# roysubhankar/dwt-domain-adaptation

Measured on NVIDIA H100. Metric: ResNet-50-DWT images/sec fwd+bwd, higher is better.
Workload: dtype f32

## Files before the change

### dwt-domain-adaptation_b200/dwt_b200/_native.py

```python
from __future__ import annotations

import ctypes
import os
import threading

import torch

_HERE = os.path.dirname(os.path.abspath(__file__))
LIB_PATH = os.environ.get("DWT_B200_LIB") or os.path.join(_HERE, "lib", "libdwt_b200.so")

ABI_VERSION = 6
MAX_DOMAINS = 4
MAX_GROUP_SIZE = 64
MODE_TRAIN, MODE_EVAL = 0, 1
EPI_NONE, EPI_AFFINE, EPI_RELU, EPI_RESIDUAL = 0, 1, 2, 4
LAYOUT_NHWC = 0x100
STATUS_NOT_PD, STATUS_BAD_LABEL = 1, 2
KIND_WHITEN, KIND_BN = 0, 1

_c_float_p = ctypes.c_void_p
_PtrArray = ctypes.c_void_p * MAX_DOMAINS


class TailSite(ctypes.Structure):
    _fields_ = [("x", ctypes.c_void_p), ("eps", ctypes.c_float), ("momentum", ctypes.c_float),
                ("update_running", ctypes.c_int), ("running_mean", ctypes.POINTER(ctypes.c_void_p)),
                ("running_cov", ctypes.POINTER(ctypes.c_void_p)), ("gamma", ctypes.c_void_p), ("beta", ctypes.c_void_p),
                ("save_mean", ctypes.c_void_p), ("save_w", ctypes.c_void_p), ("dx", ctypes.c_void_p),
                ("dgamma", ctypes.c_void_p), ("dbeta", ctypes.c_void_p)]

_SIGNATURES = {
    "dwt_abi_version": (ctypes.c_int, []),
    "dwt_last_error": (ctypes.c_char_p, []),
    "dwt_workspace_bytes": (ctypes.c_size_t, [ctypes.c_int64, ctypes.c_int64, ctypes.c_int64, ctypes.c_int, ctypes.c_int]),
    "dwt_whiten_fwd": (ctypes.c_int, [_c_float_p, _c_float_p, ctypes.c_int64, ctypes.c_int64, ctypes.c_int64,
                                      ctypes.c_int, ctypes.c_int, ctypes.c_int, ctypes.c_float, ctypes.c_float,
                                      ctypes.c_int, ctypes.POINTER(ctypes.c_void_p), ctypes.POINTER(ctypes.c_void_p),
                                      _c_float_p, _c_float_p, _c_float_p, ctypes.c_void_p, ctypes.c_int, _c_float_p,
                                      _c_float_p, ctypes.c_void_p, ctypes.c_size_t, ctypes.c_void_p]),
    "dwt_whiten_bwd": (ctypes.c_int, [_c_float_p, _c_float_p, _c_float_p, _c_float_p, ctypes.c_int64, ctypes.c_int64,
                                      ctypes.c_int64, ctypes.c_int, ctypes.c_int, ctypes.c_int, ctypes.c_float,
                                      _c_float_p, _c_float_p, _c_float_p, _c_float_p, ctypes.c_void_p, _c_float_p,
                                      ctypes.c_int, _c_float_p, _c_float_p, ctypes.c_void_p, ctypes.c_size_t,
                                      ctypes.c_void_p]),
    "dwt_bn_fwd": (ctypes.c_int, [_c_float_p, _c_float_p, ctypes.c_int64, ctypes.c_int64, ctypes.c_int64,
                                  ctypes.c_int, ctypes.c_int, ctypes.c_float, ctypes.c_float, ctypes.c_int,
                                  ctypes.POINTER(ctypes.c_void_p), ctypes.POINTER(ctypes.c_void_p), _c_float_p,
                                  _c_float_p, _c_float_p, ctypes.c_void_p, ctypes.c_int, _c_float_p, _c_float_p,
                                  ctypes.c_void_p, ctypes.c_size_t, ctypes.c_void_p]),
    "dwt_bn_bwd": (ctypes.c_int, [_c_float_p, _c_float_p, _c_float_p, _c_float_p, ctypes.c_int64, ctypes.c_int64, ctypes.c_int64,
                                  ctypes.c_int, ctypes.c_int, _c_float_p, _c_float_p, _c_float_p, _c_float_p,
                                  ctypes.c_void_p, _c_float_p, ctypes.c_int, _c_float_p, _c_float_p, ctypes.c_void_p,
                                  ctypes.c_size_t, ctypes.c_void_p]),
    "dwt_tail2_fwd": (ctypes.c_int, [ctypes.c_int, ctypes.POINTER(TailSite), _c_float_p, ctypes.c_void_p, ctypes.c_int64,
                                     ctypes.c_int64, ctypes.c_int64, ctypes.c_int, ctypes.c_int, ctypes.c_void_p,
                                     ctypes.c_size_t, ctypes.c_void_p]),
    "dwt_tail2_bwd": (ctypes.c_int, [ctypes.c_int, ctypes.POINTER(TailSite), _c_float_p, _c_float_p, ctypes.c_void_p,
                                     _c_float_p, ctypes.c_int64, ctypes.c_int64, ctypes.c_int64, ctypes.c_int, ctypes.c_int,
                                     ctypes.c_void_p, ctypes.c_size_t, ctypes.c_void_p]),
    "dwt_mec_fwd_bwd": (ctypes.c_int, [_c_float_p, _c_float_p, ctypes.c_int64, ctypes.c_int64, _c_float_p,
                                       _c_float_p, _c_float_p, ctypes.c_void_p]),
    "dwt_head_loss_fwd_bwd": (ctypes.c_int, [_c_float_p, ctypes.c_void_p, ctypes.c_int64, ctypes.c_int64, ctypes.c_float,
                                             _c_float_p, _c_float_p, ctypes.c_void_p, ctypes.c_void_p]),
    "dwt_augment_pair": (ctypes.c_int, [ctypes.c_void_p, ctypes.c_int64, ctypes.c_int, ctypes.c_int, ctypes.c_int,
                                        ctypes.c_void_p, ctypes.c_void_p, ctypes.c_void_p, _c_float_p,
                                        ctypes.POINTER(ctypes.c_float), ctypes.POINTER(ctypes.c_float), _c_float_p,
                                        _c_float_p, ctypes.c_int, ctypes.c_void_p]),
    "dwt_maxpool_fwd": (ctypes.c_int, [_c_float_p, _c_float_p, ctypes.c_void_p, ctypes.c_int64, ctypes.c_int64, ctypes.c_int64,
                                       ctypes.c_int64, ctypes.c_int, ctypes.c_int, ctypes.c_int, ctypes.c_void_p]),
    "dwt_maxpool_bwd": (ctypes.c_int, [_c_float_p, ctypes.c_void_p, _c_float_p, ctypes.c_int64, ctypes.c_int64, ctypes.c_int64,
                                       ctypes.c_int64, ctypes.c_int, ctypes.c_int, ctypes.c_int, ctypes.c_void_p]),
    "dwt_launch_count": (ctypes.c_int64, []),
    "dwt_profile_begin": (None, []),
    "dwt_profile_end": (ctypes.c_int, [ctypes.c_void_p, ctypes.c_int]),
}


class ProfileEntry(ctypes.Structure):
    _fields_ = [("name", ctypes.c_char * 48), ("launches", ctypes.c_int64), ("ms", ctypes.c_double),
                ("bytes", ctypes.c_double)]


def profile_begin():
    lib().dwt_profile_begin()


def profile_end():
    cap = 1024
    buf = (ProfileEntry * cap)()
    k = lib().dwt_profile_end(ctypes.cast(buf, ctypes.c_void_p), cap)
    return {buf[i].name.decode(): dict(launches=buf[i].launches, ms=buf[i].ms, bytes=buf[i].bytes) for i in range(k)}


def by_family(prof):
    out = {}
    for name, v in prof.items():
        f = out.setdefault(name.split("|")[0], dict(launches=0, ms=0.0, bytes=0.0))
        for k in f:
            f[k] += v[k]
    return out


def launch_count() -> int:
    return int(lib().dwt_launch_count())
EXPORTS = tuple(_SIGNATURES)

_lib = None
_lock = threading.Lock()


class NativeError(RuntimeError):
    pass


def lib() -> ctypes.CDLL:
    global _lib
    if _lib is None:
        with _lock:
            if _lib is None:
                if not os.path.exists(LIB_PATH):
                    raise NativeError(
                        f"{LIB_PATH} is missing: build it with `python {os.path.join(_HERE, 'build.py')}` "
                        "(dwt_b200 has no CPU or PyTorch fallback)")
                handle = ctypes.CDLL(LIB_PATH)
                for name, (res, args) in _SIGNATURES.items():
                    fn = getattr(handle, name)
                    fn.restype, fn.argtypes = res, args
                if handle.dwt_abi_version() != ABI_VERSION:
                    raise NativeError("libdwt_b200.so ABI version mismatch; rebuild it")
                _lib = handle
    return _lib


def channels_last_supported(channels: int, group_size: int) -> bool:
    if group_size not in (1, 2, 4) or channels % 4:
        return False
    c4 = channels // 4
    return c4 & (c4 - 1) == 0


def check(rc: int) -> None:
    if rc != 0:
        raise NativeError(f"libdwt_b200 error {rc}: {lib().dwt_last_error().decode()}")


def ptr(t):
    return None if t is None else ctypes.c_void_p(t.data_ptr())


def ptr_array(tensors):
    arr = _PtrArray()
    for i, t in enumerate(tensors):
        arr[i] = None if t is None else t.data_ptr()
    return ctypes.cast(arr, ctypes.POINTER(ctypes.c_void_p))


def require_cuda(*tensors, any_dtype=False) -> torch.device:
    dev = None
    for t in tensors:
        if t is None:
            continue
        if not t.is_cuda:
            raise NativeError("dwt_b200 runs on CUDA tensors only (no CPU fallback); got a tensor on " + str(t.device))
        if t.dtype != torch.float32 and not any_dtype:
            raise NativeError("dwt_b200 computes in float32; got " + str(t.dtype))
        if dev is None:
            dev = t.device
        elif t.device != dev:
            raise NativeError(f"tensors on different devices: {dev} vs {t.device}")
    return dev


def stream_ptr(device) -> ctypes.c_void_p:
    return ctypes.c_void_p(torch.cuda.current_stream(device).cuda_stream)


_workspaces: dict = {}


def workspace(device, n, c, hw, gs, nd):
    need = lib().dwt_workspace_bytes(n, c, hw, gs, nd)
    if need == 0:
        raise NativeError(f"invalid geometry for workspace: C={c} group_size={gs} domains={nd}")
    key = (device.index, torch.cuda.current_stream(device).cuda_stream)
    buf = _workspaces.get(key)
    if buf is None or buf.numel() < need:
        buf = torch.zeros(max(need, 8 << 20), dtype=torch.uint8, device=device)
        _workspaces[key] = buf
    return buf


def status(device=None) -> int:
    device = torch.device("cuda", torch.cuda.current_device()) if device is None else device
    buf = _workspaces.get((device.index, torch.cuda.current_stream(device).cuda_stream))
    return 0 if buf is None else int(buf[:4].view(torch.int32).item())


def status_all(device=None) -> int:
    device = torch.device("cuda", torch.cuda.current_device()) if device is None else device
    torch.cuda.synchronize(device)
    st = 0
    for (idx, _), buf in _workspaces.items():
        if idx == device.index:
            st |= int(buf[:4].view(torch.int32).item())
    return st


def status_ptr(device):
    return ctypes.c_void_p(workspace(device, 1, 4, 1, 1, 1).data_ptr())


def clear_status(device=None) -> None:
    device = torch.device("cuda", torch.cuda.current_device()) if device is None else device
    buf = _workspaces.get((device.index, torch.cuda.current_stream(device).cuda_stream))
    if buf is not None:
        buf[:4].zero_()


class NotPositiveDefiniteError(torch.linalg.LinAlgError):
    """What the reference's torch.cholesky raises at utils/whitening.py:53, raised late: the kernels never sync the
    host, so the failure is seen at the next poll (raise_on_status) or explicit check_status() call."""


_poll = {"every": 0, "count": 0}


def raise_on_status(every: int = 1) -> None:
    _poll["every"], _poll["count"] = max(0, int(every)), 0


def check_status(device=None) -> None:
    st = status(device)
    if st == 0:
        return
    clear_status(device)
    if st & STATUS_NOT_PD:
        raise NotPositiveDefiniteError(
            "cholesky: a whitening covariance was not positive definite (status word bit 0; the reference raises "
            "from torch.cholesky, utils/whitening.py:53); the affected group's output is NaN and its running-"
            "statistics update was skipped")
    if st & STATUS_BAD_LABEL:
        raise IndexError("head loss: a label was outside [0, num_classes) and is not ignore_index=-100 "
                         "(F.nll_loss asserts here); the row was dropped")
    raise NativeError(f"unknown status bits {st:#x}")


def poll_status(device) -> None:
    if _poll["every"]:
        _poll["count"] += 1
        if _poll["count"] >= _poll["every"]:
            _poll["count"] = 0
            check_status(device)
```

### dwt-domain-adaptation_b200/dwt_b200/csrc/api.cu

```cuda
#include <stdarg.h>
#include <stdio.h>
#include <stdlib.h>

#include <atomic>
#include <mutex>
#include <string>
#include <vector>
#include <string.h>

#include "norm_launch.h"

namespace {

thread_local char g_err[512] = "";

int fail(int code, const char* fmt, ...) {
  va_list ap;
  va_start(ap, fmt);
  vsnprintf(g_err, sizeof(g_err), fmt, ap);
  va_end(ap);
  return code;
}

int check_launch(const char* what) {
  cudaError_t e = cudaPeekAtLastError();
  if (e != cudaSuccess) {
    cudaGetLastError();
    return fail(DWT_E_LAUNCH, "%s: %s", what, cudaGetErrorString(e));
  }
  return DWT_OK;
}

int sm_count() {
  static int n = 0;
  if (n == 0) {
    int dev = 0;
    if (cudaGetDevice(&dev) != cudaSuccess ||
        cudaDeviceGetAttribute(&n, cudaDevAttrMultiProcessorCount, dev) != cudaSuccess || n <= 0)
      n = 132;
  }
  return n;
}

std::atomic<int64_t> g_launches{0};
std::mutex g_prof_mu;
bool g_prof_on = false;
struct ProfRec { char name[48]; cudaEvent_t a, b; double bytes; };
std::vector<ProfRec> g_prof;
std::vector<cudaEvent_t> g_event_pool;

cudaEvent_t take_event() {
  if (!g_event_pool.empty()) { cudaEvent_t e = g_event_pool.back(); g_event_pool.pop_back(); return e; }
  cudaEvent_t e = nullptr;
  cudaEventCreate(&e);
  return e;
}

struct Launch {
  cudaStream_t st; ProfRec rec; bool on;
  Launch(const char* family, const dwt::Geom* gm, double bytes, cudaStream_t s) : st(s), on(false) {
    rec.a = rec.b = nullptr; rec.bytes = bytes;
    if (gm) snprintf(rec.name, sizeof(rec.name), "%s|%d|%d|%d|%d|%d", family, gm->C, gm->HW, gm->GS, gm->D, gm->N);
    else snprintf(rec.name, sizeof(rec.name), "%s", family);
    g_launches.fetch_add(1, std::memory_order_relaxed);
    std::lock_guard<std::mutex> lk(g_prof_mu);
    if (g_prof_on && g_prof.size() < (1u << 18)) {
      on = true; rec.a = take_event(); rec.b = take_event();
      cudaEventRecord(rec.a, st);
    }
  }
  ~Launch() {
    if (!on) return;
    cudaEventRecord(rec.b, st);
    std::lock_guard<std::mutex> lk(g_prof_mu);
    g_prof.push_back(rec);
  }
};

std::once_flag g_tiled_once;
int g_tiled_rc = 0;
int ensure_tiled() {
  std::call_once(g_tiled_once, [] { g_tiled_rc = dwt::tiled_init(); });
  return g_tiled_rc;
}

std::once_flag g_tc_once;
int g_tc_rc = 0;
int ensure_tc() {
  std::call_once(g_tc_once, [] { g_tc_rc = dwt::tc_init(); });
  return g_tc_rc;
}

int tc_chunks(const dwt::Geom& g) {
  const int problems = dwt::tc_superblocks(g) * g.D;
  int n = 2 * sm_count() / problems;
  const int64_t tiles = (int64_t)g.N * ((g.HW + 31) / 32);
  if (n > tiles) n = (int)tiles;
  return n < 1 ? 1 : n;
}

int tc_apply_ctas(const dwt::Geom& g, int per_sm, int tile_px) {
  const int problems = dwt::tc_superblocks(g) * g.D;
  int n = per_sm * sm_count() / problems;
  const int64_t tiles = (int64_t)g.N * ((g.HW + tile_px - 1) / tile_px);
  if (n > tiles) n = (int)tiles;
  return n < 1 ? 1 : n;
}

int env_int(const char* name, int dflt) {
  const char* v = getenv(name);
  return (v && *v) ? atoi(v) : dflt;
}

struct ClPlan { int nred, new_, S, gridy, gz_red, gz_ew; };
ClPlan cl_plan(const dwt::Geom& g, int slots_red, int slots_ew, int unroll_red, int unroll_ew) {
  static const int seq_mb = env_int("DWT_CL_SEQ_MB", 1 << 30);
  const int C4 = g.C / 4, CW = C4 < 256 ? C4 : 256, rpi = 256 / CW, gridy = C4 / CW;
  const long long rows = (long long)g.N * g.HW;
  const double mbytes = 4.0 * (double)g.D * (double)rows * (double)g.C / 1048576.0;
  const bool seq = g.D > 1 && mbytes >= (double)seq_mb;
  ClPlan p;
  p.gridy = gridy;
  p.gz_red = p.gz_ew = seq ? 1 : g.D;
  auto shape = [&](int slots, int unroll, int gz) {
    long long by_work = rows / ((long long)rpi * unroll * 2);
    if (by_work < 1) by_work = 1;
    int cap = slots * sm_count() / (gridy * gz);
    if (cap < 1) cap = 1;
    return (int)(by_work < cap ? by_work : cap);
  };
  p.nred = shape(slots_red, unroll_red, p.gz_red);
  p.new_ = shape(slots_ew, unroll_ew, p.gz_ew);
  p.S = p.nred < 8 ? p.nred : 8;
  return p;
}

inline size_t align_up(size_t v, size_t a) { return (v + a - 1) / a * a; }

enum KernelKind { K_STATS, K_APPLY, K_BWD_REDUCE, K_BWD_APPLY };

int slots_per_sm(KernelKind k, int GS) {
  if (GS > 4) return 2;
  return ((k == K_STATS || k == K_APPLY) && GS < 4) ? 4 : 3;
}

int chunk_cap(int GS, int G, int D) {
  (void)GS;
  const int target = 16 * sm_count();
  int cap = (target + G * D - 1) / (G * D);
  return cap < 1 ? 1 : cap;
}

struct Workspace {
  int* status;
  int* counters;
  int* dom_counter;
  int* dom_counter2;
  float* partial;
  float* save_cov;
  float* coef;
  float* dgb_part;
  float* gram;
  float* shift;
  float* red;
  int* bad;
  size_t bytes;
};

constexpr size_t kMaxGroups = 65536;
constexpr size_t kOffCounters = 256;
constexpr size_t kOffDom1 = kOffCounters + sizeof(int) * DWT_MAX_DOMAINS * kMaxGroups;
constexpr size_t kOffDom2 = kOffDom1 + sizeof(int) * kMaxGroups;
constexpr size_t kOffScratch = kOffDom2 + sizeof(int) * kMaxGroups;

Workspace carve(void* base, int64_t C, int GS, int D, size_t start = kOffScratch) {
  const int G = (int)(C / GS);
  const int cap = chunk_cap(GS, G, D);
  size_t off = start;
  auto take = [&](size_t nbytes) { size_t o = off; off = align_up(off + nbytes, 256); return o; };
  char* b = static_cast<char*>(base);
  Workspace w;
  w.status = reinterpret_cast<int*>(b);
  w.counters = reinterpret_cast<int*>(b + kOffCounters);
  w.dom_counter = reinterpret_cast<int*>(b + kOffDom1);
  w.dom_counter2 = reinterpret_cast<int*>(b + kOffDom2);
  size_t partial_floats = (size_t)D * G * cap * (GS * GS + GS);
  if (GS >= 8 && 64 % GS == 0) {
    const size_t tc = ((size_t)2 * sm_count() + (size_t)((C + 63) / 64) * D) * (64 * 64 + 64);
    if (tc > partial_floats) partial_floats = tc;
  }
  size_t red_floats = 1;
  if (dwt::cl_supports((int)C, GS)) {
    const size_t W = (size_t)dwt::cl_bwd_width((int)C, GS);
    const int C4 = (int)C / 4, gridy = C4 <= 256 ? 1 : C4 / 256;
    const size_t cl = (size_t)D * (3 * sm_count() / gridy + 1) * W;
    if (cl > partial_floats) partial_floats = cl;
    red_floats = (size_t)D * 8 * W;
  }
  w.partial = reinterpret_cast<float*>(b + take(sizeof(float) * partial_floats));
  w.red = reinterpret_cast<float*>(b + take(sizeof(float) * red_floats));
  w.save_cov = reinterpret_cast<float*>(b + take(sizeof(float) * (size_t)D * G * GS * GS));
  w.coef = reinterpret_cast<float*>(b + take(sizeof(float) * (size_t)D * G * dwt::coef_stride(GS)));
  w.dgb_part = reinterpret_cast<float*>(b + take(sizeof(float) * (size_t)D * 2 * C));
  const size_t SBn = (size_t)((C + 63) / 64);
  w.gram = reinterpret_cast<float*>(b + take(sizeof(float) * (size_t)D * SBn * (64 * 64 + 64)));
  w.shift = reinterpret_cast<float*>(b + take(sizeof(float) * (size_t)D * SBn * 64));
  w.bad = reinterpret_cast<int*>(b + take(sizeof(int) * (size_t)D * G));
  w.bytes = off;
  return w;
}

struct Plan {
  dwt::Geom gm;
  dwt::Geom gm_ew;
  int vec;
  int chunks_ew;
  bool small;
};

void shape(dwt::Geom& g, int64_t work_units, KernelKind kind, bool small, int* chunks) {
  const bool reduce = (kind == K_STATS || kind == K_BWD_REDUCE);
  const int slots = slots_per_sm(kind, g.GS) * sm_count();
  const int target = reduce ? slots : 4 * slots;
  g.ppc = 1;
  if (small) {
    while (g.ppc < 8 && (int64_t)((g.G + g.ppc - 1) / g.ppc) * g.D > target) g.ppc <<= 1;
  }
  int n = 1;
  if (g.ppc == 1) {
    n = target / (g.G * g.D);
    const int cap = chunk_cap(g.GS, g.G, g.D);
    if (n > cap) n = cap;
    if (n > work_units) n = (int)work_units;
    if (n < 1) n = 1;
  }
  *chunks = n;
}

int make_plan(Plan& p, KernelKind reduce_kind, KernelKind ew_kind, const void* a0, const void* a1, const void* a2,
              int64_t N, int64_t C, int64_t HW, int GS, int D) {
  if (N <= 0 || C <= 0 || HW <= 0) return fail(DWT_E_INVALID, "empty tensor (N=%lld C=%lld HW=%lld)", (long long)N,
                                               (long long)C, (long long)HW);
  if (GS < 1 || GS > DWT_MAX_GROUP_SIZE) return fail(DWT_E_UNSUPPORTED, "group_size %d outside [1,%d]", GS,
                                                     DWT_MAX_GROUP_SIZE);
  if (C % GS != 0) return fail(DWT_E_INVALID, "channels %lld not divisible by group_size %d", (long long)C, GS);
  if (D < 1 || D > DWT_MAX_DOMAINS) return fail(DWT_E_INVALID, "n_domains %d outside [1,%d]", D, DWT_MAX_DOMAINS);
  if (N * C * HW >= (int64_t)1 << 31 || C / GS > 65535)
    return fail(DWT_E_UNSUPPORTED, "shape too large for 32-bit item indexing");
  dwt::Geom& g = p.gm;
  g.N = (int)N; g.C = (int)C; g.HW = (int)HW; g.GS = GS; g.G = (int)(C / GS); g.D = D;
  g.M = (float)((double)N * (double)HW);
  const uintptr_t bits = (uintptr_t)a0 | (uintptr_t)a1 | (uintptr_t)a2;
  p.vec = (HW % 4 == 0 && bits % 16 == 0) ? 4 : 1;
  p.small = dwt::small_supports(GS);
  int64_t work_units;
  if (p.small) work_units = (N * (HW / p.vec) + dwt::kThreads * 2 - 1) / (dwt::kThreads * 2);
  else work_units = (N * HW + 127) / 128;
  if (work_units < 1) work_units = 1;
  shape(g, work_units, reduce_kind, p.small, &g.nchunks);
  p.gm_ew = g;
  shape(p.gm_ew, work_units, ew_kind, p.small, &p.chunks_ew);
  p.gm_ew.nchunks = g.nchunks;
  return DWT_OK;
}

int check_running(bool need_running, float* const* rmean, float* const* rcov, int D) {
  if (!need_running) return DWT_OK;
  if (!rmean || !rcov) return fail(DWT_E_INVALID, "running buffers required");
  for (int d = 0; d < D; ++d)
    if (!rmean[d] || !rcov[d]) return fail(DWT_E_INVALID, "running buffer of domain %d is null", d);
  return DWT_OK;
}

dwt::FwdFin make_fwd_fin(float a, float b, float momentum, float unbias, int update_running, bool need_running,
                         float* const* rmean, float* const* rcov, float* save_mean, float* save_w, const Workspace& w, int D) {
  dwt::FwdFin fin{};
  fin.a = a; fin.b = b; fin.momentum = momentum; fin.unbias = unbias;
  fin.update_running = update_running;
  fin.save_mean = save_mean; fin.save_w = save_w; fin.save_cov = w.save_cov;
  for (int d = 0; d < D; ++d) { fin.rmean[d] = need_running ? rmean[d] : nullptr; fin.rcov[d] = need_running ? rcov[d] : nullptr; }
  fin.dom_counter = w.dom_counter; fin.status = w.status; fin.bad = w.bad;
  if (need_running && D > 1) {
    bool all_same = true, all_distinct = true;
    for (int d = 1; d < D; ++d) {
      if (rmean[d] != rmean[0] || rcov[d] != rcov[0]) all_same = false;
      for (int e = 0; e < d; ++e)
        if (rmean[d] == rmean[e] || rcov[d] == rcov[e]) all_distinct = false;
    }
    fin.aliased = all_same ? 1 : (all_distinct ? 0 : -1);
  }
  return fin;
}

dwt::BwdFin make_bwd_fin(float a, int mode, int epi, const float* save_mean, const float* save_w, const float* gamma,
                         float* dgamma, float* dbeta, const Workspace& w) {
  dwt::BwdFin fin{};
  fin.a = a; fin.mode = mode; fin.epi = epi;
  fin.save_mean = save_mean; fin.save_w = save_w; fin.gamma = gamma;
  fin.coef = w.coef; fin.dgb_part = w.dgb_part;
  fin.dgamma = (epi & DWT_EPI_AFFINE) ? dgamma : nullptr;
  fin.dbeta = (epi & DWT_EPI_AFFINE) ? dbeta : nullptr;
  fin.dom_counter = w.dom_counter2;
  return fin;
}

int whiten_like_fwd(const float* x, float* y, int64_t N, int64_t C, int64_t HW, int GS, int D, int mode, float a,
                    float b, float momentum, float unbias, int update_running, float* const* rmean,
                    float* const* rcov, const float* gamma, const float* beta, const float* residual,
                    uint8_t* relu_mask, int epi, float* save_mean, float* save_w, void* ws, size_t ws_bytes,
                    cudaStream_t st) {
  const bool nhwc = (mode & DWT_LAYOUT_NHWC) != 0;
  mode &= 0xFF;
  Plan p;
  if (int rc = make_plan(p, K_STATS, K_APPLY, x, y, nullptr, N, C, HW, GS, D)) return rc;
  if (!x || !y || !save_mean || !save_w || !ws) return fail(DWT_E_INVALID, "null pointer argument");
  if (nhwc && !dwt::cl_supports((int)C, GS))
    return fail(DWT_E_UNSUPPORTED, "channels-last layout is built for group_size 1, 2, 4 with C/4 a power of two (C=%lld gs=%d)", (long long)C, GS);
  if (nhwc && (((uintptr_t)x | (uintptr_t)y) % 16 != 0)) return fail(DWT_E_INVALID, "channels-last tensors must be 16-byte aligned");
  if (mode != DWT_MODE_TRAIN && mode != DWT_MODE_EVAL) return fail(DWT_E_INVALID, "bad mode %d", mode);
  if ((epi & DWT_EPI_RELU) && !(epi & DWT_EPI_AFFINE)) return fail(DWT_E_INVALID, "RELU epilogue needs AFFINE");
  if ((epi & DWT_EPI_AFFINE) && (!gamma || !beta)) return fail(DWT_E_INVALID, "AFFINE epilogue needs gamma and beta");
  if ((epi & DWT_EPI_RESIDUAL) && ((epi & 3) != 3 || !residual)) return fail(DWT_E_INVALID, "RESIDUAL epilogue needs AFFINE|RELU and a residual tensor");
  if ((epi & DWT_EPI_RESIDUAL) && (uintptr_t)residual % 16 != 0) return fail(DWT_E_INVALID, "residual must be 16-byte aligned");
  if (relu_mask && !((epi & DWT_EPI_RESIDUAL) && nhwc))
    return fail(DWT_E_UNSUPPORTED, "the ReLU byte map is written by the channels-last RESIDUAL epilogue only");
  if (epi != 0 && !p.small)
    return fail(DWT_E_UNSUPPORTED, "fused gamma/beta/ReLU epilogue is built for group_size 1, 2, 4 (got %d)", GS);
  const bool need_running = (mode == DWT_MODE_EVAL) || update_running;
  if (int rc = check_running(need_running, rmean, rcov, D)) return rc;
  Workspace w = carve(ws, C, GS, D);
  if (w.bytes > ws_bytes) return fail(DWT_E_WORKSPACE, "workspace too small: need %zu bytes, got %zu", w.bytes, ws_bytes);
  if ((uintptr_t)ws % 256 != 0) return fail(DWT_E_WORKSPACE, "workspace must be 256-byte aligned");
  if (!p.small && ensure_tiled() != 0) return fail(DWT_E_LAUNCH, "cudaFuncSetAttribute failed (%d)", g_tiled_rc);

  const dwt::FwdFin fin = make_fwd_fin(a, b, momentum, unbias, mode == DWT_MODE_TRAIN ? update_running : 0, need_running,
                                       rmean, rcov, save_mean, save_w, w, D);

  const double E = 4.0 * (double)D * (double)N * (double)C * (double)HW;
  if (nhwc) {
    const ClPlan cp = cl_plan(p.gm, 3, 3, 8, (epi & DWT_EPI_RESIDUAL) ? 4 : 8);
    if (mode == DWT_MODE_TRAIN) {
      {
        Launch l("cl_stats", &p.gm, E, st);
        dwt::cl_stats(x, p.gm, cp.nred, cp.gz_red, w.partial, w.shift, st);
      }
      if (int rc = check_launch("channels-last statistics kernel")) return rc;
      Launch l("cl_fwd_finalize", &p.gm, 0.0, st);
      dwt::cl_fwd_finalize(w.partial, cp.nred, w.shift, p.gm, fin, st);
    } else {
      Launch l("eval_prep", &p.gm, 0.0, st);
      dwt::small_eval_prep(p.gm, fin, st);
    }
    if (int rc = check_launch("channels-last finalize kernel")) return rc;
    {
      Launch l("cl_apply", &p.gm, ((epi & DWT_EPI_RESIDUAL) ? (relu_mask ? 3.0625 : 3.0) : 2.0) * E, st);
      dwt::cl_apply(x, y, p.gm, cp.new_, cp.gz_ew, epi, save_mean, save_w, gamma, beta, residual, relu_mask, st);
    }
    return check_launch("channels-last apply kernel");
  }
  const bool tc = !p.small && dwt::tc_supports(p.gm, p.vec) && ensure_tc() == 0;
  if (mode == DWT_MODE_TRAIN) {
    Launch l(p.small ? "small_stats" : (tc ? "tc_stats" : "tiled_stats"), &p.gm, E, st);
    if (p.small) dwt::small_stats(x, p.gm, p.vec, fin, w.partial, w.counters, st);
    else if (tc) {
      if (int cr = dwt::tc_stats(x, p.gm, tc_chunks(p.gm), w.shift, w.partial, st))
        return fail(DWT_E_LAUNCH, "cuTensorMapEncodeTiled failed (CUresult %d) x=%p N=%d C=%d HW=%d D=%d", cr, (const void*)x, p.gm.N, p.gm.C, p.gm.HW, p.gm.D);
    } else dwt::tiled_stats(x, p.gm, p.vec, fin, w.partial, w.counters, st);
  } else {
    Launch l("eval_prep", &p.gm, 0.0, st);
    if (p.small) dwt::small_eval_prep(p.gm, fin, st);
    else if (tc) dwt::dense_fwd_factor(nullptr, nullptr, p.gm, fin, st);
    else dwt::tiled_eval_prep(p.gm, fin, st);
  }
  if (tc && mode == DWT_MODE_TRAIN) {
    if (int rc = check_launch("tensor-core statistics kernel")) return rc;
    Launch l("dense_fwd_finalize", &p.gm, 0.0, st);
    dwt::dense_partial_reduce(w.partial, tc_chunks(p.gm), dwt::tc_superblocks(p.gm) * D, w.gram, st);
    dwt::dense_fwd_factor(w.gram, w.shift, p.gm, fin, st);
  }
  if (int rc = check_launch("whitening statistics kernel")) return rc;
  {
    Launch l(p.small ? "small_apply" : (tc ? "tc_apply" : "tiled_apply"), &p.gm, ((epi & DWT_EPI_RESIDUAL) ? 3 : 2) * E, st);
    if (p.small) dwt::small_apply(x, y, p.gm_ew, p.vec, p.chunks_ew, epi, save_mean, save_w, gamma, beta, residual, st);
    else if (tc) {
      if (int cr = dwt::tc_apply(x, y, p.gm, tc_apply_ctas(p.gm, 1, 64), save_mean, save_w, st))
        return fail(DWT_E_LAUNCH, "cuTensorMapEncodeTiled failed (CUresult %d)", cr);
    } else dwt::tiled_apply(x, y, p.gm_ew, p.vec, p.chunks_ew, save_mean, save_w, st);
  }
  return check_launch("whitening apply kernel");
}

int whiten_like_bwd(const float* x, const float* dout, const float* dout2, float* dx, int64_t N, int64_t C, int64_t HW, int GS, int D,
                    int mode, float a, const float* save_mean, const float* save_w, const float* gamma,
                    const float* beta, const uint8_t* relu_mask, float* dresidual, int epi, float* dgamma,
                    float* dbeta, void* ws, size_t ws_bytes, cudaStream_t st) {
  const bool nhwc = (mode & DWT_LAYOUT_NHWC) != 0;
  mode &= 0xFF;
  Plan p;
  if (int rc = make_plan(p, K_BWD_REDUCE, K_BWD_APPLY, x, dout, dx, N, C, HW, GS, D)) return rc;
  if (!x || !dout || !dx || !save_mean || !save_w || !ws) return fail(DWT_E_INVALID, "null pointer argument");
  if (dout2 && (!nhwc || (uintptr_t)dout2 % 16 != 0))
    return fail(nhwc ? DWT_E_INVALID : DWT_E_UNSUPPORTED, "a second gradient addend (dout2) is built for the channels-last "
                "kernels (16-byte aligned tensor); add it to dout otherwise");
  if (nhwc && !dwt::cl_supports((int)C, GS))
    return fail(DWT_E_UNSUPPORTED, "channels-last layout is built for group_size 1, 2, 4 with C/4 a power of two (C=%lld gs=%d)", (long long)C, GS);
  if (nhwc && (((uintptr_t)x | (uintptr_t)dout | (uintptr_t)dx) % 16 != 0)) return fail(DWT_E_INVALID, "channels-last tensors must be 16-byte aligned");
  if (mode != DWT_MODE_TRAIN && mode != DWT_MODE_EVAL) return fail(DWT_E_INVALID, "bad mode %d", mode);
  if ((epi & DWT_EPI_RELU) && !(epi & DWT_EPI_AFFINE)) return fail(DWT_E_INVALID, "RELU epilogue needs AFFINE");
  if ((epi & DWT_EPI_AFFINE) && (!gamma || !beta)) return fail(DWT_E_INVALID, "AFFINE epilogue needs gamma and beta");
  if (epi & DWT_EPI_RESIDUAL) {
    if (!nhwc || !relu_mask || (epi & 3) != 3 || !dresidual)
      return fail(DWT_E_INVALID, "backward of a RESIDUAL forward needs the channels-last layout, AFFINE|RELU, the forward's "
                                 "ReLU byte map and dresidual (or pass dout already masked by (out > 0) with epilogue AFFINE)");
    if ((uintptr_t)dresidual % 16 != 0) return fail(DWT_E_INVALID, "dresidual must be 16-byte aligned");
  } else if (relu_mask || dresidual) {
    return fail(DWT_E_INVALID, "relu_mask / dresidual belong to the RESIDUAL epilogue");
  }
  if ((dgamma == nullptr) != (dbeta == nullptr)) return fail(DWT_E_INVALID, "dgamma and dbeta go together");
  if (epi != 0 && !p.small)
    return fail(DWT_E_UNSUPPORTED, "fused gamma/beta/ReLU epilogue is built for group_size 1, 2, 4 (got %d)", GS);
  Workspace w = carve(ws, C, GS, D);
  if (w.bytes > ws_bytes) return fail(DWT_E_WORKSPACE, "workspace too small: need %zu bytes, got %zu", w.bytes, ws_bytes);
  if ((uintptr_t)ws % 256 != 0) return fail(DWT_E_WORKSPACE, "workspace must be 256-byte aligned");
  if (!p.small && ensure_tiled() != 0) return fail(DWT_E_LAUNCH, "cudaFuncSetAttribute failed (%d)", g_tiled_rc);

  const dwt::BwdFin fin = make_bwd_fin(a, mode, epi, save_mean, save_w, gamma, dgamma, dbeta, w);
  const bool masked = nhwc && (epi & DWT_EPI_RESIDUAL) != 0;

  const bool need_reduce = (mode == DWT_MODE_TRAIN) || (fin.dgamma != nullptr) || masked;
  const double E = 4.0 * (double)D * (double)N * (double)C * (double)HW;
  if (nhwc) {
    const ClPlan cp = cl_plan(p.gm, 2, 2, 4, 4);
    if (need_reduce) {
      {
        Launch l("cl_bwd_reduce", &p.gm, ((masked ? 3.0625 : 2.0) + (dout2 ? 1.0 : 0.0)) * E, st);
        dwt::cl_bwd_reduce(x, dout, dout2, p.gm, cp.nred, cp.gz_red, epi, save_mean, save_w, gamma, beta, relu_mask, dresidual, w.partial, st);
      }
      if (int rc = check_launch("channels-last backward reduction kernel")) return rc;
      Launch l("cl_bwd_finalize", &p.gm, 0.0, st);
      dwt::cl_bwd_finalize(w.partial, cp.nred, p.gm, fin, st);
    } else {
      Launch l("bwd_prep", &p.gm, 0.0, st);
      dwt::small_bwd_prep(p.gm, fin, st);
    }
    if (int rc = check_launch("channels-last backward finalize kernel")) return rc;
    {
      Launch l("cl_bwd_apply", &p.gm, (3.0 + (dout2 && !masked ? 1.0 : 0.0)) * E, st);
      if (masked) dwt::cl_bwd_apply(x, dresidual, nullptr, dx, p.gm, cp.new_, cp.gz_ew, DWT_EPI_AFFINE, w.coef, save_mean, save_w, gamma, beta, st);
      else dwt::cl_bwd_apply(x, dout, dout2, dx, p.gm, cp.new_, cp.gz_ew, epi, w.coef, save_mean, save_w, gamma, beta, st);
    }
    return check_launch("channels-last backward apply kernel");
  }
  const bool tc = !p.small && dwt::tc_supports(p.gm, p.vec) && ensure_tc() == 0;
  if (need_reduce) {
    Launch l(p.small ? "small_bwd_reduce" : (tc ? "tc_bwd_reduce" : "tiled_bwd_reduce"), &p.gm, 2 * E, st);
    if (p.small) dwt::small_bwd_reduce(x, dout, p.gm, p.vec, fin, beta, w.partial, w.counters, st);
    else if (tc) {
      if (int cr = dwt::tc_bwd_reduce(x, dout, p.gm, tc_chunks(p.gm), save_mean, w.partial, st))
        return fail(DWT_E_LAUNCH, "cuTensorMapEncodeTiled failed (CUresult %d) x=%p dout=%p N=%d C=%d HW=%d D=%d", cr, (const void*)x, (const void*)dout, p.gm.N, p.gm.C, p.gm.HW, p.gm.D);
    } else dwt::tiled_bwd_reduce(x, dout, p.gm, p.vec, fin, w.partial, w.counters, st);
  } else {
    Launch l("bwd_prep", &p.gm, 0.0, st);
    if (p.small) dwt::small_bwd_prep(p.gm, fin, st);
    else if (tc) dwt::dense_bwd_coef(nullptr, p.gm, fin, w.shift, st);
    else dwt::tiled_bwd_prep(p.gm, fin, st);
  }
  if (tc && need_reduce) {
    if (int rc = check_launch("tensor-core backward reduction kernel")) return rc;
    Launch l("dense_bwd_finalize", &p.gm, 0.0, st);
    dwt::dense_partial_reduce(w.partial, tc_chunks(p.gm), dwt::tc_superblocks(p.gm) * D, w.gram, st);
    dwt::dense_bwd_coef(w.gram, p.gm, fin, w.shift, st);
  }
  if (int rc = check_launch("whitening backward reduction kernel")) return rc;
  {
    Launch l(p.small ? "small_bwd_apply" : (tc ? "tc_bwd_apply" : "tiled_bwd_apply"), &p.gm, 3 * E, st);
    if (p.small) dwt::small_bwd_apply(x, dout, dx, p.gm_ew, p.vec, p.chunks_ew, epi, w.coef, save_mean, save_w, gamma, beta, st);
    else if (tc) {
      if (int cr = dwt::tc_bwd_apply(x, dout, dx, p.gm, tc_apply_ctas(p.gm, 1, 64), w.coef, save_mean, w.shift, st))
        return fail(DWT_E_LAUNCH, "cuTensorMapEncodeTiled failed (CUresult %d)", cr);
    } else dwt::tiled_bwd_apply(x, dout, dx, p.gm_ew, p.vec, p.chunks_ew, w.coef, st);
  }
  return check_launch("whitening backward apply kernel");
}

struct SiteConst { float a, b, unbias; };
SiteConst site_const(int kind, float eps, int64_t N, int64_t HW) {
  if (kind == DWT_KIND_BN) {
    const double M = (double)N * (double)HW;
    return {1.f, eps, M > 1.0 ? (float)(M / (M - 1.0)) : 1.f};
  }
  return {1.f - eps, eps, 1.f};
}

int tail2_plan(Plan& p, int kind, const dwt_tail_site* s, const void* out, int64_t N, int64_t C, int64_t HW, int GS, int D) {
  if (kind != DWT_KIND_WHITEN && kind != DWT_KIND_BN) return fail(DWT_E_INVALID, "bad kind %d", kind);
  if (kind == DWT_KIND_BN && GS != 1) return fail(DWT_E_INVALID, "batch norm has group_size 1 (got %d)", GS);
  if (!s) return fail(DWT_E_INVALID, "null pointer argument");
  if (int rc = make_plan(p, K_STATS, K_APPLY, s[0].x, s[1].x, out, N, C, HW, GS, D)) return rc;
  if (!dwt::cl_supports((int)C, GS))
    return fail(DWT_E_UNSUPPORTED, "the two-site tail runs on the channels-last kernels: group_size 1, 2, 4 with C/4 a power of two (C=%lld gs=%d)",
                (long long)C, GS);
  for (int k = 0; k < 2; ++k)
    if (!s[k].x || !s[k].gamma || !s[k].beta || !s[k].save_mean || !s[k].save_w || !out) return fail(DWT_E_INVALID, "null pointer argument");
  if ((((uintptr_t)s[0].x | (uintptr_t)s[1].x | (uintptr_t)out) % 16) != 0) return fail(DWT_E_INVALID, "channels-last tensors must be 16-byte aligned");
  return DWT_OK;
}

int tail2_workspace(Workspace (&w)[2], void* ws, size_t ws_bytes, int64_t C, int GS, int D) {
  if (!ws) return fail(DWT_E_INVALID, "null pointer argument");
  w[0] = carve(ws, C, GS, D);
  w[1] = carve(ws, C, GS, D, w[0].bytes);
  if (w[1].bytes > ws_bytes) return fail(DWT_E_WORKSPACE, "workspace too small: need %zu bytes, got %zu", w[1].bytes, ws_bytes);
  if ((uintptr_t)ws % 256 != 0) return fail(DWT_E_WORKSPACE, "workspace must be 256-byte aligned");
  return DWT_OK;
}

int tail2_fwd(int kind, const dwt_tail_site* s, float* y, uint8_t* relu_mask, int64_t N, int64_t C, int64_t HW, int GS, int D,
              void* ws, size_t ws_bytes, cudaStream_t st) {
  Plan p;
  if (int rc = tail2_plan(p, kind, s, y, N, C, HW, GS, D)) return rc;
  if (!relu_mask) return fail(DWT_E_INVALID, "the two-site tail writes the ReLU byte map its backward reads");
  for (int k = 0; k < 2; ++k)
    if (int rc = check_running(s[k].update_running != 0, s[k].running_mean, s[k].running_cov, D)) return rc;
  Workspace w[2];
  if (int rc = tail2_workspace(w, ws, ws_bytes, C, GS, D)) return rc;
  dwt::FwdFin fin[2];
  for (int k = 0; k < 2; ++k) {
    const SiteConst sc = site_const(kind, s[k].eps, N, HW);
    fin[k] = make_fwd_fin(sc.a, sc.b, s[k].momentum, sc.unbias, s[k].update_running, s[k].update_running != 0, s[k].running_mean,
                          s[k].running_cov, s[k].save_mean, s[k].save_w, w[k], D);
  }
  const double E = 4.0 * (double)D * (double)N * (double)C * (double)HW;
  const ClPlan cp = cl_plan(p.gm, 3, 3, 8, 4);
  for (int k = 0; k < 2; ++k) {
    Launch l("cl_stats", &p.gm, E, st);
    dwt::cl_stats(s[k].x, p.gm, cp.nred, cp.gz_red, w[k].partial, w[k].shift, st);
  }
  if (int rc = check_launch("channels-last statistics kernel")) return rc;
  {
    Launch l("cl_tail2_fwd_finalize", &p.gm, 0.0, st);
    dwt::cl_fwd_finalize(w[0].partial, cp.nred, w[0].shift, p.gm, fin[0], st, &fin[1], (size_t)(w[1].partial - w[0].partial),
                         (size_t)(w[1].shift - w[0].shift));
  }
  if (int rc = check_launch("channels-last finalize kernel")) return rc;
  {
    Launch l("cl_tail2_apply", &p.gm, 3.0625 * E, st);
    dwt::cl_tail2_apply(s[0].x, s[1].x, y, p.gm, cp.new_, cp.gz_ew, s[0].save_mean, s[0].save_w, s[0].gamma, s[0].beta,
                        s[1].save_mean, s[1].save_w, s[1].gamma, s[1].beta, relu_mask, st);
  }
  return check_launch("channels-last two-site apply kernel");
}

int tail2_bwd(int kind, const dwt_tail_site* s, const float* dout, const float* dout2, const uint8_t* relu_mask, float* dz,
              int64_t N, int64_t C, int64_t HW, int GS, int D, void* ws, size_t ws_bytes, cudaStream_t st) {
  Plan p;
  if (int rc = tail2_plan(p, kind, s, dz, N, C, HW, GS, D)) return rc;
  if (!dout || !relu_mask || !s[0].dx || !s[1].dx) return fail(DWT_E_INVALID, "null pointer argument");
  if ((((uintptr_t)dout | (uintptr_t)dout2 | (uintptr_t)s[0].dx | (uintptr_t)s[1].dx) % 16) != 0)
    return fail(DWT_E_INVALID, "channels-last tensors must be 16-byte aligned");
  for (int k = 0; k < 2; ++k)
    if ((s[k].dgamma == nullptr) != (s[k].dbeta == nullptr)) return fail(DWT_E_INVALID, "dgamma and dbeta go together");
  Workspace w[2];
  if (int rc = tail2_workspace(w, ws, ws_bytes, C, GS, D)) return rc;
  dwt::BwdFin fin[2];
  for (int k = 0; k < 2; ++k)
    fin[k] = make_bwd_fin(site_const(kind, s[k].eps, N, HW).a, DWT_MODE_TRAIN, k ? DWT_EPI_AFFINE : (DWT_EPI_AFFINE | DWT_EPI_RELU | DWT_EPI_RESIDUAL),
                          s[k].save_mean, s[k].save_w, s[k].gamma, s[k].dgamma, s[k].dbeta, w[k]);
  const double E = 4.0 * (double)D * (double)N * (double)C * (double)HW;
  const ClPlan cp = cl_plan(p.gm, 2, 2, 4, 4);
  {
    Launch l("cl_tail2_bwd_reduce", &p.gm, (4.0625 + (dout2 ? 1.0 : 0.0)) * E, st);
    dwt::cl_tail2_bwd_reduce(s[0].x, s[1].x, dout, dout2, p.gm, cp.nred, cp.gz_red, s[0].save_mean, s[1].save_mean, relu_mask, dz,
                             w[0].partial, (size_t)(w[1].partial - w[0].partial), st);
  }
  if (int rc = check_launch("channels-last two-site backward reduction kernel")) return rc;
  {
    Launch l("cl_tail2_bwd_finalize", &p.gm, 0.0, st);
    dwt::cl_bwd_finalize(w[0].partial, cp.nred, p.gm, fin[0], st, &fin[1], (size_t)(w[1].partial - w[0].partial));
  }
  if (int rc = check_launch("channels-last backward finalize kernel")) return rc;
  {
    Launch l("cl_tail2_bwd_apply", &p.gm, 5.0 * E, st);
    dwt::cl_tail2_bwd_apply(s[0].x, s[1].x, dz, s[0].dx, s[1].dx, p.gm, cp.new_, cp.gz_ew, w[0].coef, w[1].coef, st);
  }
  return check_launch("channels-last two-site backward apply kernel");
}

}

extern "C" {

int dwt_abi_version(void) { return DWT_B200_ABI_VERSION; }

const char* dwt_last_error(void) { return g_err; }

size_t dwt_workspace_bytes(int64_t N, int64_t C, int64_t HW, int group_size, int n_domains) {
  (void)N; (void)HW;
  if (C <= 0 || group_size < 1 || group_size > DWT_MAX_GROUP_SIZE || C % group_size != 0 || n_domains < 1 ||
      n_domains > DWT_MAX_DOMAINS)
    return 0;
  return carve(nullptr, C, group_size, n_domains, carve(nullptr, C, group_size, n_domains).bytes).bytes;
}

int dwt_whiten_fwd(const float* x, float* y, int64_t N, int64_t C, int64_t HW, int group_size, int n_domains,
                   int mode, float eps, float momentum, int update_running, float* const* running_mean,
                   float* const* running_cov, const float* gamma, const float* beta, const float* residual,
                   uint8_t* relu_mask, int epilogue, float* save_mean, float* save_w, void* workspace,
                   size_t workspace_bytes, dwt_stream_t stream) {
  return whiten_like_fwd(x, y, N, C, HW, group_size, n_domains, mode, 1.f - eps, eps, momentum, 1.f, update_running,
                         running_mean, running_cov, gamma, beta, residual, relu_mask, epilogue, save_mean, save_w,
                         workspace, workspace_bytes, (cudaStream_t)stream);
}

int dwt_whiten_bwd(const float* x, const float* dout, const float* dout2, float* dx, int64_t N, int64_t C, int64_t HW, int group_size,
                   int n_domains, int mode, float eps, const float* save_mean, const float* save_w,
                   const float* gamma, const float* beta, const uint8_t* relu_mask, float* dresidual, int epilogue,
                   float* dgamma, float* dbeta, void* workspace, size_t workspace_bytes, dwt_stream_t stream) {
  return whiten_like_bwd(x, dout, dout2, dx, N, C, HW, group_size, n_domains, mode, 1.f - eps, save_mean, save_w, gamma,
                         beta, relu_mask, dresidual, epilogue, dgamma, dbeta, workspace, workspace_bytes,
                         (cudaStream_t)stream);
}

int dwt_bn_fwd(const float* x, float* y, int64_t N, int64_t C, int64_t HW, int n_domains, int mode, float eps,
               float factor, int update_running, float* const* running_mean, float* const* running_var,
               const float* weight, const float* bias, const float* residual, uint8_t* relu_mask, int epilogue,
               float* save_mean, float* save_invstd, void* workspace, size_t workspace_bytes, dwt_stream_t stream) {
  const double M = (double)N * (double)HW;
  const float unbias = M > 1.0 ? (float)(M / (M - 1.0)) : 1.f;
  return whiten_like_fwd(x, y, N, C, HW, 1, n_domains, mode, 1.f, eps, factor, unbias, update_running, running_mean,
                         running_var, weight, bias, residual, relu_mask, epilogue, save_mean, save_invstd, workspace,
                         workspace_bytes, (cudaStream_t)stream);
}

int dwt_bn_bwd(const float* x, const float* dout, const float* dout2, float* dx, int64_t N, int64_t C, int64_t HW, int n_domains,
               int mode, const float* save_mean, const float* save_invstd, const float* weight, const float* bias,
               const uint8_t* relu_mask, float* dresidual, int epilogue, float* dweight, float* dbias, void* workspace,
               size_t workspace_bytes, dwt_stream_t stream) {
  return whiten_like_bwd(x, dout, dout2, dx, N, C, HW, 1, n_domains, mode, 1.f, save_mean, save_invstd, weight, bias,
                         relu_mask, dresidual, epilogue, dweight, dbias, workspace, workspace_bytes,
                         (cudaStream_t)stream);
}

int dwt_tail2_fwd(int kind, const dwt_tail_site* sites, float* y, uint8_t* relu_mask, int64_t N, int64_t C, int64_t HW,
                  int group_size, int n_domains, void* workspace, size_t workspace_bytes, dwt_stream_t stream) {
  return tail2_fwd(kind, sites, y, relu_mask, N, C, HW, group_size, n_domains, workspace, workspace_bytes, (cudaStream_t)stream);
}

int dwt_tail2_bwd(int kind, const dwt_tail_site* sites, const float* dout, const float* dout2, const uint8_t* relu_mask, float* dz,
                  int64_t N, int64_t C, int64_t HW, int group_size, int n_domains, void* workspace, size_t workspace_bytes,
                  dwt_stream_t stream) {
  return tail2_bwd(kind, sites, dout, dout2, relu_mask, dz, N, C, HW, group_size, n_domains, workspace, workspace_bytes,
                   (cudaStream_t)stream);
}

int dwt_mec_fwd_bwd(const float* x, const float* y, int64_t N, int64_t K, float* loss, float* gx, float* gy,
                    dwt_stream_t stream) {
  if (!x || !y || !loss || !gx || !gy) return fail(DWT_E_INVALID, "null pointer argument");
  if (N <= 0 || K <= 0 || N >= (1 << 24) || K >= (1 << 24)) return fail(DWT_E_INVALID, "bad logits shape [%lld,%lld]", (long long)N, (long long)K);
  {
    Launch l("mec", nullptr, 16.0 * (double)N * (double)K, (cudaStream_t)stream);
    dwt::mec_launch(x, y, (int)N, (int)K, loss, gx, gy, (cudaStream_t)stream);
  }
  return check_launch("MEC kernel");
}

int dwt_head_loss_fwd_bwd(const float* logits, const int64_t* labels, int64_t B, int64_t K, float lambda, float* losses,
                          float* grad, int* status, dwt_stream_t stream) {
  if (!logits || !labels || !losses || !grad) return fail(DWT_E_INVALID, "null pointer argument");
  if (B <= 0 || K <= 0 || B >= (1 << 22) || K >= (1 << 24)) return fail(DWT_E_INVALID, "bad logits shape [3*%lld,%lld]", (long long)B, (long long)K);
  {
    Launch l("head_loss", nullptr, 4.0 * 3 * (double)B * (double)K * 2, (cudaStream_t)stream);
    dwt::head_loss_launch(logits, reinterpret_cast<const long long*>(labels), (int)B, (int)K, lambda, losses, grad, status,
                          (cudaStream_t)stream);
  }
  return check_launch("head loss kernel");
}

int dwt_augment_pair(const uint8_t* images, int64_t B, int src_h, int src_w, int crop, const int32_t* crop_plain,
                     const int32_t* crop_aug, const uint8_t* flip, const float* affine, const float* mean,
                     const float* stdv, float* out_plain, float* out_aug, int layout, dwt_stream_t stream) {
  if (!images || !mean || !stdv) return fail(DWT_E_INVALID, "null pointer argument");
  if (!out_plain && !out_aug) return fail(DWT_E_INVALID, "at least one of out_plain / out_aug is needed");
  if (out_plain && !crop_plain) return fail(DWT_E_INVALID, "out_plain needs crop_plain");
  if (out_aug && (!crop_aug || !flip || !affine)) return fail(DWT_E_INVALID, "out_aug needs crop_aug, flip and affine");
  if (B <= 0 || B > 65535 || src_h <= 0 || src_w <= 0 || src_h > 16384 || src_w > 16384)
    return fail(DWT_E_INVALID, "bad image batch [%lld,%d,%d,3]", (long long)B, src_h, src_w);
  if (crop <= 0 || crop > src_h || crop > src_w) return fail(DWT_E_INVALID, "crop %d does not fit %dx%d", crop, src_h, src_w);
  if (layout != 0 && layout != DWT_LAYOUT_NHWC) return fail(DWT_E_INVALID, "layout must be 0 (NCHW) or DWT_LAYOUT_NHWC");
  for (int c = 0; c < 3; ++c)
    if (!(stdv[c] != 0.f)) return fail(DWT_E_INVALID, "std[%d] must be non-zero", c);
  {
    const double px = (double)B * crop * crop;
    Launch l("augment_pair", nullptr, px * 3 * ((out_plain ? 5.0 : 0.0) + (out_aug ? 5.0 : 0.0)), (cudaStream_t)stream);
    dwt::augment_pair_launch(images, (int)B, src_h, src_w, crop, crop_plain, crop_aug, flip, affine, mean, stdv, out_plain,
                             out_aug, layout != 0, (cudaStream_t)stream);
  }
  return check_launch("augmentation kernel");
}

namespace {
int pool_check(int64_t N, int64_t H, int64_t W, int64_t C, int k, int s, int p, int* OH, int* OW) {
  if (N <= 0 || H <= 0 || W <= 0 || C <= 0 || C % 4 != 0) return fail(DWT_E_INVALID, "bad pooling input [%lld,%lld,%lld,%lld] (C must be a multiple of 4)", (long long)N, (long long)H, (long long)W, (long long)C);
  if (k < 1 || k > 15 || s < 1 || p < 0 || 2 * p > k) return fail(DWT_E_INVALID, "bad pooling window k=%d s=%d p=%d (k <= 15, pad <= k/2)", k, s, p);
  if (H + 2 * p < k || W + 2 * p < k) return fail(DWT_E_INVALID, "pooling window larger than the padded image");
  *OH = (int)((H + 2 * p - k) / s + 1);
  *OW = (int)((W + 2 * p - k) / s + 1);
  if (N * H * W * C >= ((int64_t)1 << 40)) return fail(DWT_E_UNSUPPORTED, "tensor too large");
  return DWT_OK;
}
}

int dwt_maxpool_fwd(const float* x, float* y, uint8_t* argmax, int64_t N, int64_t H, int64_t W, int64_t C, int kernel,
                    int stride, int padding, dwt_stream_t stream) {
  int OH = 0, OW = 0;
  if (int rc = pool_check(N, H, W, C, kernel, stride, padding, &OH, &OW)) return rc;
  if (!x || !y || !argmax) return fail(DWT_E_INVALID, "null pointer argument");
  if ((((uintptr_t)x | (uintptr_t)y) % 16) != 0 || (uintptr_t)argmax % 4 != 0) return fail(DWT_E_INVALID, "pooling tensors must be 16-byte aligned");
  {
    const double in = (double)N * H * W * C, out = (double)N * OH * OW * C;
    Launch l("maxpool_fwd", nullptr, 4.0 * (in + out) + out, (cudaStream_t)stream);
    dwt::maxpool_fwd_launch(x, y, argmax, (int)N, (int)H, (int)W, (int)C, OH, OW, kernel, stride, padding, (cudaStream_t)stream);
  }
  return check_launch("max-pool forward kernel");
}

int dwt_maxpool_bwd(const float* dy, const uint8_t* argmax, float* dx, int64_t N, int64_t H, int64_t W, int64_t C, int kernel,
                    int stride, int padding, dwt_stream_t stream) {
  int OH = 0, OW = 0;
  if (int rc = pool_check(N, H, W, C, kernel, stride, padding, &OH, &OW)) return rc;
  if (!dy || !dx || !argmax) return fail(DWT_E_INVALID, "null pointer argument");
  if ((((uintptr_t)dy | (uintptr_t)dx) % 16) != 0 || (uintptr_t)argmax % 4 != 0) return fail(DWT_E_INVALID, "pooling tensors must be 16-byte aligned");
  {
    const double in = (double)N * H * W * C, out = (double)N * OH * OW * C;
    Launch l("maxpool_bwd", nullptr, 4.0 * (in + out) + out, (cudaStream_t)stream);
    dwt::maxpool_bwd_launch(dy, argmax, dx, (int)N, (int)H, (int)W, (int)C, OH, OW, kernel, stride, padding, (cudaStream_t)stream);
  }
  return check_launch("max-pool backward kernel");
}

int64_t dwt_launch_count(void) { return g_launches.load(); }

void dwt_profile_begin(void) {
  std::lock_guard<std::mutex> lk(g_prof_mu);
  for (auto& r : g_prof) { g_event_pool.push_back(r.a); g_event_pool.push_back(r.b); }
  g_prof.clear();
  g_prof_on = true;
}

int dwt_profile_end(dwt_profile_entry* out, int max_entries) {
  std::vector<ProfRec> recs;
  {
    std::lock_guard<std::mutex> lk(g_prof_mu);
    g_prof_on = false;
    recs.swap(g_prof);
  }
  int n = 0;
  for (auto& r : recs) {
    float ms = 0.f;
    if (cudaEventSynchronize(r.b) == cudaSuccess && cudaEventElapsedTime(&ms, r.a, r.b) == cudaSuccess) {
      int k = 0;
      for (; k < n; ++k)
        if (strcmp(out[k].name, r.name) == 0) break;
      if (k == n && n < max_entries) {
        memset(&out[n], 0, sizeof(out[n]));
        strncpy(out[n].name, r.name, sizeof(out[n].name) - 1);
        ++n;
      }
      if (k < n) { out[k].launches += 1; out[k].ms += ms; out[k].bytes += r.bytes; }
    }
    std::lock_guard<std::mutex> lk(g_prof_mu);
    g_event_pool.push_back(r.a); g_event_pool.push_back(r.b);
  }
  return n;
}

}
```

### dwt-domain-adaptation_b200/dwt_b200/csrc/norm_cl.cu

```cuda
#include <stdlib.h>

#include "dwt_common.cuh"
#include "norm_launch.h"
#include "small_algebra.cuh"

namespace dwt {
namespace {

constexpr int kT = 256;

__device__ __forceinline__ void pdl_wait() { asm volatile("griddepcontrol.wait;" ::: "memory"); }
__device__ __forceinline__ void pdl_launch_dependents() { asm volatile("griddepcontrol.launch_dependents;" ::: "memory"); }

template <int GS> struct ClShape {
  static constexpr int NSUB = 4 / GS;
  static constexpr int NM = GS * (GS + 1) / 2;
  static constexpr int FWD1 = GS + NM;
  static constexpr int BWD1 = GS * GS + GS;
  static constexpr int FWD = NSUB * FWD1;
  static constexpr int BWD = NSUB * BWD1;
};

struct ClThread {
  int C4, CW, rpi, col, rsub, q;
  __device__ __forceinline__ ClThread(const Geom& gm) {
    C4 = gm.C >> 2;
    CW = C4 < kT ? C4 : kT;
    rpi = kT / CW;
    col = threadIdx.x % CW;
    rsub = threadIdx.x / CW;
    q = blockIdx.y * CW + col;
  }
};

template <int UNROLL, bool DESC, class F>
__device__ __forceinline__ void sweep_rows(const ClThread& t, unsigned rows, F&& body) {
  const unsigned krows = (unsigned)t.rpi * UNROLL, nch = (rows + krows - 1) / krows;
  for (unsigned i = blockIdx.x; i < nch; i += gridDim.x) body((DESC ? nch - 1 - i : i) * krows + t.rsub);
}
#define CL_FOR_DOMAINS(d, gm, DESC) \
  for (int di_ = blockIdx.z, d = (DESC) ? (gm).D - 1 - di_ : di_; di_ < (gm).D; di_ += gridDim.z, d = (DESC) ? (gm).D - 1 - di_ : di_)

__device__ __forceinline__ float4 ldg4(const float* p) { return __ldg(reinterpret_cast<const float4*>(p)); }

template <int NACC>
__device__ __forceinline__ void column_reduce(const ClThread& t, float (&acc)[NACC], float* sRed) {
  if (t.rpi == 1) return;
#pragma unroll
  for (int i = 0; i < NACC; ++i) sRed[i * kT + threadIdx.x] = acc[i];
  __syncthreads();
  if (t.rsub == 0) {
#pragma unroll
    for (int i = 0; i < NACC; ++i) {
      float s = acc[i];
      for (int r = 1; r < t.rpi; ++r) s += sRed[i * kT + r * t.CW + t.col];
      acc[i] = s;
    }
  }
}

template <int GS>
__global__ void __launch_bounds__(kT, 3) cl_stats_kernel(const float* __restrict__ x, const Geom gm,
                                                         float* __restrict__ partial, float* __restrict__ shift) {
  using S = ClShape<GS>;
  constexpr int UNROLL = 8;
  __shared__ float sRed[kT * S::FWD];
  const ClThread t(gm);
  const unsigned rows = (unsigned)gm.N * gm.HW;
  pdl_launch_dependents();
  CL_FOR_DOMAINS(d, gm, true) {
    const float* xd = x + (size_t)d * rows * gm.C + 4 * t.q;
    float K[4] = {0.f, 0.f, 0.f, 0.f};
    {
      const unsigned np = rows < 8 ? rows : 8;
      for (unsigned r = 0; r < np; ++r) {
        const float4 v = ldg4(xd + (size_t)r * gm.C);
        K[0] += v.x; K[1] += v.y; K[2] += v.z; K[3] += v.w;
      }
#pragma unroll
      for (int c = 0; c < 4; ++c) K[c] /= (float)np;
      if (blockIdx.x == 0 && t.rsub == 0) *reinterpret_cast<float4*>(shift + (size_t)d * gm.C + 4 * t.q) = make_float4(K[0], K[1], K[2], K[3]);
    }
    float acc[S::FWD];
#pragma unroll
    for (int i = 0; i < S::FWD; ++i) acc[i] = 0.f;
    sweep_rows<UNROLL, true>(t, rows, [&](unsigned r) {
      float4 v[UNROLL];
#pragma unroll
      for (int u = 0; u < UNROLL; ++u) {
        const unsigned rr = r + u * t.rpi;
        v[u] = rr < rows ? ldg4(xd + (size_t)rr * gm.C) : make_float4(K[0], K[1], K[2], K[3]);
      }
#pragma unroll
      for (int u = 0; u < UNROLL; ++u) {
        const float e[4] = {v[u].x - K[0], v[u].y - K[1], v[u].z - K[2], v[u].w - K[3]};
#pragma unroll
        for (int s = 0; s < S::NSUB; ++s) {
#pragma unroll
          for (int c = 0; c < GS; ++c) {
            acc[s * S::FWD1 + c] += e[s * GS + c];
#pragma unroll
            for (int j = 0; j <= c; ++j)
              acc[s * S::FWD1 + GS + c * (c + 1) / 2 + j] = fmaf(e[s * GS + c], e[s * GS + j], acc[s * S::FWD1 + GS + c * (c + 1) / 2 + j]);
          }
        }
      }
    });
    column_reduce<S::FWD>(t, acc, sRed);
    if (t.rsub == 0) {
      float* dst = partial + (((size_t)d * gridDim.x + blockIdx.x) * t.C4 + t.q) * S::FWD;
#pragma unroll
      for (int i = 0; i < S::FWD; ++i) dst[i] = acc[i];
    }
    if (gridDim.z == 1) __syncthreads();
  }
}

template <int GS, int PER>
__device__ __forceinline__ int acc_index(int g, int a) {
  constexpr int NSUB = 4 / GS;
  return (g / NSUB) * (NSUB * PER) + (g % NSUB) * PER + a;
}

constexpr int kFinQ = 2;

template <int NACC>
__device__ __forceinline__ void column_row_sum(const float* __restrict__ col, int nrows, int W, float (&a)[NACC]) {
  static_assert(NACC % 2 == 0, "accumulators are read as float2");
#pragma unroll
  for (int i = 0; i < NACC; ++i) a[i] = 0.f;
#pragma unroll 4
  for (int r = threadIdx.x; r < nrows; r += 32) {
    const float2* p = reinterpret_cast<const float2*>(col + (size_t)r * W);
#pragma unroll
    for (int i = 0; i < NACC / 2; ++i) {
      const float2 v = __ldcg(p + i);
      a[2 * i] += v.x; a[2 * i + 1] += v.y;
    }
  }
#pragma unroll
  for (int o = 1; o < 32; o <<= 1)
#pragma unroll
    for (int i = 0; i < NACC; ++i) a[i] += __shfl_xor_sync(0xffffffffu, a[i], o);
}

template <int NSUB, int PER>
__device__ __forceinline__ void take_group(const float (&a)[NSUB * PER], int s, float (&v)[PER]) {
#pragma unroll
  for (int i = 0; i < PER; ++i) {
    v[i] = a[i];
#pragma unroll
    for (int k = 1; k < NSUB; ++k)
      if (s == k) v[i] = a[k * PER + i];
  }
}

template <int GS>
__device__ __forceinline__ void cl_fwd_finalize_site(const float* __restrict__ partial, int nrows, const float* __restrict__ shift,
                                                     const Geom& gm, const FwdFin& fin) {
  using SH = ClShape<GS>;
  constexpr int NST = GS + GS * GS;
  __shared__ float sStat[DWT_MAX_DOMAINS][kFinQ][SH::NSUB][NST + 1];
  __shared__ unsigned char sBad[DWT_MAX_DOMAINS][kFinQ][SH::NSUB];
  const int s = threadIdx.x, ql = threadIdx.y, d = threadIdx.z, q = blockIdx.x * blockDim.y + ql;
  const int W = (gm.C >> 2) * SH::FWD;
  const float invM = 1.f / gm.M;
  const bool lead = s < SH::NSUB;
  const int g = q * SH::NSUB + (lead ? s : 0);
  const bool direct = gm.D == 1 || fin.aliased == 0;
  const int dbuf = direct ? d : 0;
  const bool upd = fin.update_running && lead && (direct || (fin.aliased == 1 && d == 0));
  float rc_old[GS * GS], rm_old[GS];
  if (upd) {
#pragma unroll
    for (int e = 0; e < GS * GS; ++e) rc_old[e] = fin.rcov[dbuf][(size_t)g * GS * GS + e];
#pragma unroll
    for (int e = 0; e < GS; ++e) rm_old[e] = fin.rmean[dbuf][g * GS + e];
  }
  pdl_launch_dependents();
  pdl_wait();
  float a[SH::FWD];
  column_row_sum<SH::FWD>(partial + (size_t)d * nrows * W + (size_t)q * SH::FWD, nrows, W, a);
  if (lead) {
    float v[SH::FWD1];
    take_group<SH::NSUB, SH::FWD1>(a, s, v);
    float mean[GS], cov[GS][GS];
#pragma unroll
    for (int i = 0; i < GS; ++i) mean[i] = shift[(size_t)d * gm.C + g * GS + i] + v[i] * invM;
#pragma unroll
    for (int i = 0; i < GS; ++i)
#pragma unroll
      for (int j = 0; j <= i; ++j) {
        const float c = v[GS + i * (i + 1) / 2 + j] * invM - (v[i] * invM) * (v[j] * invM);
        cov[i][j] = c; cov[j][i] = c;
      }
    const bool bad = factor_thread<GS>(gm, fin, d, g, mean, cov, false);
    if (fin.update_running) {
      if (direct) {
        if (!bad) {
          const float m = fin.momentum, kk = 1.f - fin.momentum;
#pragma unroll
          for (int i = 0; i < GS; ++i) {
            fin.rmean[d][g * GS + i] = m * mean[i] + kk * rm_old[i];
#pragma unroll
            for (int j = 0; j < GS; ++j)
              fin.rcov[d][(size_t)g * GS * GS + i * GS + j] = m * (cov[i][j] * fin.unbias) + kk * rc_old[i * GS + j];
          }
        }
      } else {
        sBad[d][ql][s] = bad ? 1 : 0;
#pragma unroll
        for (int i = 0; i < GS; ++i) {
          sStat[d][ql][s][i] = mean[i];
#pragma unroll
          for (int j = 0; j < GS; ++j) sStat[d][ql][s][GS + i * GS + j] = cov[i][j];
        }
      }
    }
  }
  if (!fin.update_running || direct) return;
  __syncthreads();
  if (!(lead && d == 0)) return;
  if (fin.aliased == 1) {
    const float m = fin.momentum, kk = 1.f - fin.momentum;
    float* rc = fin.rcov[0] + (size_t)g * GS * GS;
    float* rm = fin.rmean[0] + g * GS;
    for (int dd = 0; dd < gm.D; ++dd) {
      if (sBad[dd][ql][s]) continue;
#pragma unroll
      for (int e = 0; e < GS * GS; ++e) rc_old[e] = m * (sStat[dd][ql][s][GS + e] * fin.unbias) + kk * rc_old[e];
#pragma unroll
      for (int e = 0; e < GS; ++e) rm_old[e] = m * sStat[dd][ql][s][e] + kk * rm_old[e];
    }
#pragma unroll
    for (int e = 0; e < GS * GS; ++e) rc[e] = rc_old[e];
#pragma unroll
    for (int e = 0; e < GS; ++e) rm[e] = rm_old[e];
  } else {
    for (int dd = 0; dd < gm.D; ++dd)
      if (!sBad[dd][ql][s]) ema_direct<GS>(gm, fin, dd, g, &sStat[dd][ql][s][0], &sStat[dd][ql][s][GS]);
  }
}

template <int GS>
__global__ void __launch_bounds__(32 * kFinQ * DWT_MAX_DOMAINS) cl_fwd_finalize_kernel(const float* __restrict__ partial, size_t pstride, int nrows,
                                                                                      const float* __restrict__ shift, size_t sstride, const Geom gm,
                                                                                      const __grid_constant__ FwdFin fin, const __grid_constant__ FwdFin fin2) {
  const bool second = blockIdx.y != 0;
  cl_fwd_finalize_site<GS>(partial + (second ? pstride : 0), nrows, shift + (second ? sstride : 0), gm, second ? fin2 : fin);
}

template <int GS, int EPI, bool DS>
__global__ void __launch_bounds__(kT, 3) cl_apply_kernel(const float* __restrict__ x, float* __restrict__ y, const Geom gm,
                                                         const float* __restrict__ save_mean, const float* __restrict__ save_w,
                                                         const float* __restrict__ gamma, const float* __restrict__ beta,
                                                         const float* __restrict__ res, uint8_t* __restrict__ mask,
                                                         const float* __restrict__ save_mean_d, const float* __restrict__ save_w_d,
                                                         const float* __restrict__ gamma_d, const float* __restrict__ beta_d) {
  using S = ClShape<GS>;
  constexpr bool RES = (EPI & DWT_EPI_RESIDUAL) != 0;
  static_assert(!DS || RES, "the two-site tail is a residual epilogue");
  constexpr int UNROLL = DS ? 2 : (RES ? 4 : 8);
  const ClThread t(gm);
  const unsigned rows = (unsigned)gm.N * gm.HW;
  pdl_wait();
  CL_FOR_DOMAINS(d, gm, false) {
    float Wp[S::NSUB][S::NM], bp[S::NSUB][GS], Wd[DS ? S::NSUB : 1][S::NM], bd[DS ? S::NSUB : 1][GS];
#pragma unroll
    for (int s = 0; s < S::NSUB; ++s) {
      const int g = t.q * S::NSUB + s;
      load_forward_map<GS, EPI>(save_w + ((size_t)d * gm.G + g) * GS * GS, save_mean + (size_t)d * gm.C + g * GS,
                                gamma + g * GS, beta + g * GS, Wp[s], bp[s]);
      if constexpr (DS)
        load_forward_map<GS, DWT_EPI_AFFINE>(save_w_d + ((size_t)d * gm.G + g) * GS * GS, save_mean_d + (size_t)d * gm.C + g * GS,
                                             gamma_d + g * GS, beta_d + g * GS, Wd[s], bd[s]);
    }
    const size_t base = (size_t)d * rows * gm.C + 4 * t.q;
    const float* xd = x + base;
    const float* rd = res + base;
    float* yd = y + base;
    uint8_t* md = mask + (size_t)d * rows * t.C4 + t.q;
    sweep_rows<UNROLL, false>(t, rows, [&](unsigned r) {
      float4 v[UNROLL], rs[UNROLL];
#pragma unroll
      for (int u = 0; u < UNROLL; ++u) {
        const unsigned rr = r + u * t.rpi;
        if (rr < rows) {
          v[u] = ldg4(xd + (size_t)rr * gm.C);
          if constexpr (RES) rs[u] = ldg4(rd + (size_t)rr * gm.C);
        }
      }
#pragma unroll
      for (int u = 0; u < UNROLL; ++u) {
        const unsigned rr = r + u * t.rpi;
        if (rr < rows) {
          const float e[4] = {v[u].x, v[u].y, v[u].z, v[u].w};
          float o[4], ra[4] = {0.f, 0.f, 0.f, 0.f};
          if constexpr (RES) { ra[0] = rs[u].x; ra[1] = rs[u].y; ra[2] = rs[u].z; ra[3] = rs[u].w; }
          unsigned bits = 0;
#pragma unroll
          for (int s = 0; s < S::NSUB; ++s) {
            float xi[GS], oi[GS];
            if constexpr (DS) {
              float xdi[GS], odi[GS];
#pragma unroll
              for (int c = 0; c < GS; ++c) xdi[c] = ra[s * GS + c];
              apply_group<GS>(Wd[s], bd[s], xdi, odi);
#pragma unroll
              for (int c = 0; c < GS; ++c) ra[s * GS + c] = odi[c];
            }
#pragma unroll
            for (int c = 0; c < GS; ++c) xi[c] = e[s * GS + c];
            apply_group<GS>(Wp[s], bp[s], xi, oi);
#pragma unroll
            for (int c = 0; c < GS; ++c) {
              const float z = RES ? oi[c] + ra[s * GS + c] : oi[c];
              if constexpr (RES) bits |= (z > 0.f ? 1u : 0u) << (s * GS + c);
              o[s * GS + c] = (EPI & DWT_EPI_RELU) ? fmaxf(z, 0.f) : z;
            }
          }
          *reinterpret_cast<float4*>(yd + (size_t)rr * gm.C) = make_float4(o[0], o[1], o[2], o[3]);
          if constexpr (RES) { if (mask != nullptr) md[(size_t)rr * t.C4] = (uint8_t)bits; }
        }
      }
    });
  }
}

template <int GS>
__device__ __forceinline__ void bwd_accumulate(float* acc, const float (&dz)[GS], const float (&xi)[GS], const float* mu) {
#pragma unroll
  for (int i = 0; i < GS; ++i) {
    acc[GS * GS + i] += dz[i];
#pragma unroll
    for (int j = 0; j < GS; ++j) acc[i * GS + j] = fmaf(dz[i], xi[j] - mu[j], acc[i * GS + j]);
  }
}

template <int GS, int EPI, bool D2, bool DS>
__global__ void __launch_bounds__(kT, 2) cl_bwd_reduce_kernel(const float* __restrict__ x, const float* __restrict__ dout, const float* __restrict__ dout2,
                                                              const Geom gm, const float* __restrict__ save_mean,
                                                              const float* __restrict__ save_w, const float* __restrict__ gamma,
                                                              const float* __restrict__ beta, const uint8_t* __restrict__ mask,
                                                              float* __restrict__ dzout, float* __restrict__ partial,
                                                              const float* __restrict__ xds, const float* __restrict__ save_mean_d,
                                                              size_t pstride) {
  using S = ClShape<GS>;
  constexpr int UNROLL = 4;
  constexpr bool MASK = (EPI & DWT_EPI_RESIDUAL) != 0;
  constexpr bool RELU = (EPI & DWT_EPI_RELU) != 0 && !MASK;
  static_assert(!DS || MASK, "the two-site tail is a residual epilogue");
  constexpr int NS = DS ? 2 : 1;
  __shared__ float sRed[kT * S::BWD];
  const ClThread t(gm);
  const unsigned rows = (unsigned)gm.N * gm.HW;
  pdl_launch_dependents();
  CL_FOR_DOMAINS(d, gm, true) {
    float Wp[S::NSUB][S::NM], bp[S::NSUB][GS], mu[NS][4];
#pragma unroll
    for (int s = 0; s < S::NSUB; ++s) {
      const int g = t.q * S::NSUB + s;
      if constexpr (RELU)
        load_forward_map<GS, EPI>(save_w + ((size_t)d * gm.G + g) * GS * GS, save_mean + (size_t)d * gm.C + g * GS,
                                  gamma + g * GS, beta + g * GS, Wp[s], bp[s]);
    }
#pragma unroll
    for (int k = 0; k < NS; ++k) {
      const float4 m4 = ldg4((k ? save_mean_d : save_mean) + (size_t)d * gm.C + 4 * t.q);
      mu[k][0] = m4.x; mu[k][1] = m4.y; mu[k][2] = m4.z; mu[k][3] = m4.w;
    }
    float acc[NS][S::BWD];
#pragma unroll
    for (int k = 0; k < NS; ++k)
#pragma unroll
      for (int i = 0; i < S::BWD; ++i) acc[k][i] = 0.f;
    const size_t base = (size_t)d * rows * gm.C + 4 * t.q;
    const float* xp[NS];
    xp[0] = x + base;
    if constexpr (DS) xp[NS - 1] = xds + base;
    const float* gd = dout + base;
    const float* gd2 = D2 ? dout2 + base : nullptr;
    float* zd = MASK ? dzout + base : nullptr;
    const uint8_t* md = mask + (size_t)d * rows * t.C4 + t.q;
    constexpr int H = DS ? UNROLL / 2 : UNROLL;
    sweep_rows<UNROLL, true>(t, rows, [&](unsigned r0) {
#pragma unroll
     for (int h = 0; h < UNROLL; h += H) {
      const unsigned r = r0 + h * t.rpi;
      float4 v[NS][H], q[H], q2[D2 ? H : 1];
      unsigned mb[H];
#pragma unroll
      for (int u = 0; u < H; ++u) {
        const unsigned rr = r + u * t.rpi;
        if (rr < rows) {
#pragma unroll
          for (int k = 0; k < NS; ++k) v[k][u] = ldg4(xp[k] + (size_t)rr * gm.C);
          q[u] = ldg4(gd + (size_t)rr * gm.C);
          if constexpr (MASK) mb[u] = __ldg(md + (size_t)rr * t.C4);
          if constexpr (D2) q2[u] = ldg4(gd2 + (size_t)rr * gm.C);
        } else {
#pragma unroll
          for (int k = 0; k < NS; ++k) v[k][u] = make_float4(mu[k][0], mu[k][1], mu[k][2], mu[k][3]);
          q[u] = make_float4(0.f, 0.f, 0.f, 0.f);
          if constexpr (MASK) mb[u] = 0u;
          if constexpr (D2) q2[u] = make_float4(0.f, 0.f, 0.f, 0.f);
        }
      }
      if constexpr (D2) {
#pragma unroll
        for (int u = 0; u < H; ++u) { q[u].x += q2[u].x; q[u].y += q2[u].y; q[u].z += q2[u].z; q[u].w += q2[u].w; }
      }
#pragma unroll
      for (int u = 0; u < H; ++u) {
        const float ge[4] = {q[u].x, q[u].y, q[u].z, q[u].w};
        const float e[4] = {v[0][u].x, v[0][u].y, v[0][u].z, v[0][u].w};
        const float ed[4] = {v[NS - 1][u].x, v[NS - 1][u].y, v[NS - 1][u].z, v[NS - 1][u].w};
        float zm[4];
#pragma unroll
        for (int s = 0; s < S::NSUB; ++s) {
          float xi[GS], dz[GS];
#pragma unroll
          for (int c = 0; c < GS; ++c) { xi[c] = e[s * GS + c]; dz[c] = ge[s * GS + c]; }
          if constexpr (RELU) {
            float oi[GS];
            apply_group<GS>(Wp[s], bp[s], xi, oi);
#pragma unroll
            for (int c = 0; c < GS; ++c) dz[c] = oi[c] > 0.f ? dz[c] : 0.f;
          }
          if constexpr (MASK) {
#pragma unroll
            for (int c = 0; c < GS; ++c) { dz[c] = ((mb[u] >> (s * GS + c)) & 1u) ? dz[c] : 0.f; zm[s * GS + c] = dz[c]; }
          }
          bwd_accumulate<GS>(acc[0] + s * S::BWD1, dz, xi, &mu[0][s * GS]);
          if constexpr (DS) {
#pragma unroll
            for (int c = 0; c < GS; ++c) xi[c] = ed[s * GS + c];
            bwd_accumulate<GS>(acc[NS - 1] + s * S::BWD1, dz, xi, &mu[NS - 1][s * GS]);
          }
        }
        if constexpr (MASK) {
          const unsigned rr = r + u * t.rpi;
          if (rr < rows) *reinterpret_cast<float4*>(zd + (size_t)rr * gm.C) = make_float4(zm[0], zm[1], zm[2], zm[3]);
        }
      }
     }
    });
#pragma unroll
    for (int k = 0; k < NS; ++k) {
      if (k) __syncthreads();
      column_reduce<S::BWD>(t, acc[k], sRed);
      if (t.rsub == 0) {
        float* dst = partial + k * pstride + (((size_t)d * gridDim.x + blockIdx.x) * t.C4 + t.q) * S::BWD;
#pragma unroll
        for (int i = 0; i < S::BWD; ++i) dst[i] = acc[k][i];
      }
    }
    if (gridDim.z == 1) __syncthreads();
  }
}

template <int GS>
__device__ __forceinline__ void cl_bwd_finalize_site(const float* __restrict__ partial, int nrows, const Geom& gm, const BwdFin& fin) {
  using SH = ClShape<GS>;
  const int s = threadIdx.x, d = threadIdx.z, q = blockIdx.x * blockDim.y + threadIdx.y;
  const int W = (gm.C >> 2) * SH::BWD;
  pdl_launch_dependents();
  pdl_wait();
  float a[SH::BWD];
  column_row_sum<SH::BWD>(partial + (size_t)d * nrows * W + (size_t)q * SH::BWD, nrows, W, a);
  if (s < SH::NSUB) {
    float v[SH::BWD1], R[GS][GS], sdz[GS];
    take_group<SH::NSUB, SH::BWD1>(a, s, v);
#pragma unroll
    for (int i = 0; i < SH::BWD1; ++i) {
      if (i < GS * GS) R[i / GS][i % GS] = v[i]; else sdz[i - GS * GS] = v[i];
    }
    bwd_finalize_thread<GS>(gm, fin, d, q * SH::NSUB + s, R, sdz, false);
  }
  if (!((fin.epi & DWT_EPI_AFFINE) && fin.dgamma != nullptr)) return;
  __syncthreads();
  if (d == 0 && s < 4) {
    const int ch = 4 * q + s;
    float sg = 0.f, sb = 0.f;
    for (int dd = 0; dd < gm.D; ++dd) {
      sg += fin.dgb_part[((size_t)dd * 2 + 0) * gm.C + ch];
      sb += fin.dgb_part[((size_t)dd * 2 + 1) * gm.C + ch];
    }
    fin.dgamma[ch] = sg;
    fin.dbeta[ch] = sb;
  }
}

template <int GS>
__global__ void __launch_bounds__(32 * kFinQ * DWT_MAX_DOMAINS) cl_bwd_finalize_kernel(const float* __restrict__ partial, size_t pstride, int nrows,
                                                                                      const Geom gm, const __grid_constant__ BwdFin fin,
                                                                                      const __grid_constant__ BwdFin fin2) {
  const bool second = blockIdx.y != 0;
  cl_bwd_finalize_site<GS>(partial + (second ? pstride : 0), nrows, gm, second ? fin2 : fin);
}

template <int GS>
struct BwdCoef {
  float A1[GS * (GS + 1) / 2], Bm[GS * (GS + 1) / 2], cv[GS];
  __device__ __forceinline__ void load(const float* cf) {
#pragma unroll
    for (int i = 0; i < GS; ++i) {
      cv[i] = __ldg(cf + 2 * GS * GS + i);
#pragma unroll
      for (int j = 0; j <= i; ++j) {
        A1[i * (i + 1) / 2 + j] = __ldg(cf + j * GS + i);
        Bm[i * (i + 1) / 2 + j] = __ldg(cf + GS * GS + i * GS + j);
      }
    }
  }
  __device__ __forceinline__ void apply(const float (&dz)[GS], const float (&xi)[GS], float* o) const {
#pragma unroll
    for (int i = 0; i < GS; ++i) {
      float a = cv[i];
#pragma unroll
      for (int j = i; j < GS; ++j) a = fmaf(A1[j * (j + 1) / 2 + i], dz[j], a);
#pragma unroll
      for (int j = 0; j < GS; ++j) {
        const int hi = i > j ? i : j, lo = i > j ? j : i;
        a = fmaf(Bm[hi * (hi + 1) / 2 + lo], xi[j], a);
      }
      o[i] = a;
    }
  }
};

template <int GS, int EPI, bool D2, bool DS>
__global__ void __launch_bounds__(kT, 2) cl_bwd_apply_kernel(const float* __restrict__ x, const float* __restrict__ dout, const float* __restrict__ dout2,
                                                             float* __restrict__ dx, const Geom gm, const float* __restrict__ coef,
                                                             const float* __restrict__ save_mean, const float* __restrict__ save_w,
                                                             const float* __restrict__ gamma, const float* __restrict__ beta,
                                                             const float* __restrict__ xds, float* __restrict__ dxds,
                                                             const float* __restrict__ coef_d) {
  using S = ClShape<GS>;
  constexpr int UNROLL = 4;
  constexpr bool RELU = (EPI & DWT_EPI_RELU) != 0;
  static_assert((EPI & DWT_EPI_RESIDUAL) == 0, "the residual tail's apply runs with EPI = AFFINE on dz");
  static_assert(!DS || (!D2 && !RELU), "the two-site tail's apply reads dz");
  constexpr int NS = DS ? 2 : 1;
  const ClThread t(gm);
  const unsigned rows = (unsigned)gm.N * gm.HW;
  pdl_wait();
  CL_FOR_DOMAINS(d, gm, false) {
    float Wp[S::NSUB][S::NM], bp[S::NSUB][GS];
    BwdCoef<GS> cf[NS][S::NSUB];
#pragma unroll
    for (int s = 0; s < S::NSUB; ++s) {
      const int g = t.q * S::NSUB + s;
      if constexpr (RELU)
        load_forward_map<GS, EPI>(save_w + ((size_t)d * gm.G + g) * GS * GS, save_mean + (size_t)d * gm.C + g * GS,
                                  gamma + g * GS, beta + g * GS, Wp[s], bp[s]);
#pragma unroll
      for (int k = 0; k < NS; ++k) cf[k][s].load((k ? coef_d : coef) + ((size_t)d * gm.G + g) * coef_stride(GS));
    }
    const size_t base = (size_t)d * rows * gm.C + 4 * t.q;
    const float* xp[NS];
    float* op[NS];
    xp[0] = x + base; op[0] = dx + base;
    if constexpr (DS) { xp[NS - 1] = xds + base; op[NS - 1] = dxds + base; }
    const float* gd = dout + base;
    const float* gd2 = D2 ? dout2 + base : nullptr;
    sweep_rows<UNROLL, false>(t, rows, [&](unsigned r) {
      float4 v[NS][UNROLL], q[UNROLL], q2[D2 ? UNROLL : 1];
#pragma unroll
      for (int u = 0; u < UNROLL; ++u) {
        const unsigned rr = r + u * t.rpi;
        if (rr < rows) {
#pragma unroll
          for (int k = 0; k < NS; ++k) v[k][u] = ldg4(xp[k] + (size_t)rr * gm.C);
          q[u] = ldg4(gd + (size_t)rr * gm.C);
          if constexpr (D2) q2[u] = ldg4(gd2 + (size_t)rr * gm.C);
        }
      }
      if constexpr (D2) {
#pragma unroll
        for (int u = 0; u < UNROLL; ++u)
          if (r + u * t.rpi < rows) { q[u].x += q2[u].x; q[u].y += q2[u].y; q[u].z += q2[u].z; q[u].w += q2[u].w; }
      }
#pragma unroll
      for (int u = 0; u < UNROLL; ++u) {
        const unsigned rr = r + u * t.rpi;
        if (rr < rows) {
          const float ge[4] = {q[u].x, q[u].y, q[u].z, q[u].w};
#pragma unroll
          for (int k = 0; k < NS; ++k) {
            const float e[4] = {v[k][u].x, v[k][u].y, v[k][u].z, v[k][u].w};
            float o[4];
#pragma unroll
            for (int s = 0; s < S::NSUB; ++s) {
              float xi[GS], dz[GS];
#pragma unroll
              for (int c = 0; c < GS; ++c) { xi[c] = e[s * GS + c]; dz[c] = ge[s * GS + c]; }
              if constexpr (RELU) {
                float oi[GS];
                apply_group<GS>(Wp[s], bp[s], xi, oi);
#pragma unroll
                for (int c = 0; c < GS; ++c) dz[c] = oi[c] > 0.f ? dz[c] : 0.f;
              }
              cf[k][s].apply(dz, xi, o + s * GS);
            }
            *reinterpret_cast<float4*>(op[k] + (size_t)rr * gm.C) = make_float4(o[0], o[1], o[2], o[3]);
          }
        }
      }
    });
  }
}

#define CL_GS(GS_, ...)                                  \
  switch (GS_) {                                         \
    case 1: { constexpr int kGS = 1; __VA_ARGS__; break; } \
    case 2: { constexpr int kGS = 2; __VA_ARGS__; break; } \
    case 4: { constexpr int kGS = 4; __VA_ARGS__; break; } \
    default: break;                                      \
  }
#define CL_EPI(E_, ...)                                                   \
  if ((E_) == 3) { constexpr int kEPI = 3; __VA_ARGS__; }                 \
  else if ((E_) == 1) { constexpr int kEPI = 1; __VA_ARGS__; }            \
  else { constexpr int kEPI = 0; __VA_ARGS__; }
#define CL_EPI_BWD(E_, ...)                                               \
  if ((E_) == 7) { constexpr int kEPI = 7; __VA_ARGS__; }                 \
  else CL_EPI(E_, __VA_ARGS__)
#define CL_D2(P_, ...)                                                    \
  if (P_) { constexpr bool kD2 = true; __VA_ARGS__; }                     \
  else { constexpr bool kD2 = false; __VA_ARGS__; }

inline bool use_pdl() {
  static const bool on = [] { const char* v = getenv("DWT_PDL"); return v != nullptr && v[0] == '1'; }();
  return on;
}

template <class... KArgs, class... Args>
inline void launch_k(void (*kernel)(KArgs...), dim3 grid, dim3 block, cudaStream_t st, bool pdl, Args... args) {
  cudaLaunchConfig_t cfg = {};
  cfg.gridDim = grid; cfg.blockDim = block; cfg.dynamicSmemBytes = 0; cfg.stream = st;
  cudaLaunchAttribute attr[1];
  attr[0].id = cudaLaunchAttributeProgrammaticStreamSerialization;
  attr[0].val.programmaticStreamSerializationAllowed = 1;
  cfg.attrs = attr; cfg.numAttrs = pdl ? 1 : 0;
  cudaLaunchKernelEx(&cfg, kernel, KArgs(args)...);
}

inline dim3 cl_grid(const Geom& gm, int nctas, int gz) {
  const int C4 = gm.C / 4, CW = C4 < kT ? C4 : kT;
  return dim3(nctas, C4 / CW, gz);
}

}

bool cl_supports(int C, int GS) {
  if (!(GS == 1 || GS == 2 || GS == 4) || C % 4 != 0) return false;
  const int c4 = C / 4;
  return (c4 & (c4 - 1)) == 0 && c4 <= 16384;
}
int cl_fwd_width(int C, int GS) { return (C / 4) * (4 / GS) * (GS + GS * (GS + 1) / 2); }
int cl_bwd_width(int C, int GS) { return (C / 4) * (4 / GS) * (GS * GS + GS); }


void cl_stats(const float* x, const Geom& gm, int nctas, int gz, float* partial, float* shift, cudaStream_t st) {
  CL_GS(gm.GS, (cl_stats_kernel<kGS><<<cl_grid(gm, nctas, gz), kT, 0, st>>>(x, gm, partial, shift)));
}
inline dim3 fin_block(const Geom& gm) { const int c4 = gm.C / 4; return dim3(32, c4 < kFinQ ? c4 : kFinQ, gm.D); }
void cl_fwd_finalize(const float* partial, int nrows, const float* shift, const Geom& gm, const FwdFin& fin, cudaStream_t st,
                     const FwdFin* fin2, size_t pstride, size_t sstride) {
  const dim3 b = fin_block(gm), g((gm.C / 4) / b.y, fin2 ? 2 : 1);
  CL_GS(gm.GS, (launch_k(cl_fwd_finalize_kernel<kGS>, g, b, st, use_pdl(), partial, pstride, nrows, shift, sstride, gm, fin, fin2 ? *fin2 : fin)));
}
void cl_apply(const float* x, float* y, const Geom& gm, int nctas, int gz, int epi, const float* mean, const float* w,
              const float* gamma, const float* beta, const float* residual, uint8_t* mask, cudaStream_t st) {
  const float* nul = nullptr;
  if (epi == 7) {
    CL_GS(gm.GS, (launch_k(cl_apply_kernel<kGS, 7, false>, cl_grid(gm, nctas, gz), dim3(kT), st, use_pdl(), x, y, gm, mean, w, gamma, beta, residual, mask,
                           nul, nul, nul, nul)));
    return;
  }
  CL_GS(gm.GS, CL_EPI(epi, (launch_k(cl_apply_kernel<kGS, kEPI, false>, cl_grid(gm, nctas, gz), dim3(kT), st, use_pdl(), x, y, gm, mean, w, gamma, beta,
                                     nul, (uint8_t*)nullptr, nul, nul, nul, nul))));
}
void cl_tail2_apply(const float* x, const float* xd, float* y, const Geom& gm, int nctas, int gz, const float* mean, const float* w,
                    const float* gamma, const float* beta, const float* mean_d, const float* w_d, const float* gamma_d,
                    const float* beta_d, uint8_t* mask, cudaStream_t st) {
  CL_GS(gm.GS, (launch_k(cl_apply_kernel<kGS, 7, true>, cl_grid(gm, nctas, gz), dim3(kT), st, use_pdl(), x, y, gm, mean, w, gamma, beta, xd, mask,
                         mean_d, w_d, gamma_d, beta_d)));
}
void cl_bwd_reduce(const float* x, const float* dout, const float* dout2, const Geom& gm, int nctas, int gz, int epi, const float* mean, const float* w,
                   const float* gamma, const float* beta, const uint8_t* mask, float* dz, float* partial, cudaStream_t st) {
  const float* nul = nullptr;
  CL_GS(gm.GS, CL_D2(dout2, CL_EPI_BWD(epi, (cl_bwd_reduce_kernel<kGS, kEPI, kD2, false><<<cl_grid(gm, nctas, gz), kT, 0, st>>>(
                                                x, dout, dout2, gm, mean, w, gamma, beta, mask, dz, partial, nul, nul, 0)))));
}
void cl_tail2_bwd_reduce(const float* x, const float* xd, const float* dout, const float* dout2, const Geom& gm, int nctas, int gz,
                         const float* mean, const float* mean_d, const uint8_t* mask, float* dz, float* partial, size_t pstride,
                         cudaStream_t st) {
  const float* nul = nullptr;
  CL_GS(gm.GS, CL_D2(dout2, (cl_bwd_reduce_kernel<kGS, 7, kD2, true><<<cl_grid(gm, nctas, gz), kT, 0, st>>>(
                                x, dout, dout2, gm, mean, nul, nul, nul, mask, dz, partial, xd, mean_d, pstride))));
}
void cl_bwd_finalize(const float* partial, int nrows, const Geom& gm, const BwdFin& fin, cudaStream_t st, const BwdFin* fin2, size_t pstride) {
  const dim3 b = fin_block(gm), g((gm.C / 4) / b.y, fin2 ? 2 : 1);
  CL_GS(gm.GS, (launch_k(cl_bwd_finalize_kernel<kGS>, g, b, st, use_pdl(), partial, pstride, nrows, gm, fin, fin2 ? *fin2 : fin)));
}
void cl_bwd_apply(const float* x, const float* dout, const float* dout2, float* dx, const Geom& gm, int nctas, int gz, int epi, const float* coef,
                  const float* mean, const float* w, const float* gamma, const float* beta, cudaStream_t st) {
  const float* nul = nullptr;
  CL_GS(gm.GS, CL_D2(dout2, CL_EPI(epi, (launch_k(cl_bwd_apply_kernel<kGS, kEPI, kD2, false>, cl_grid(gm, nctas, gz), dim3(kT), st, use_pdl(), x, dout,
                                                  dout2, dx, gm, coef, mean, w, gamma, beta, nul, (float*)nullptr, nul)))));
}
void cl_tail2_bwd_apply(const float* x, const float* xd, const float* dz, float* dx, float* dxd, const Geom& gm, int nctas, int gz,
                        const float* coef, const float* coef_d, cudaStream_t st) {
  const float* nul = nullptr;
  CL_GS(gm.GS, (launch_k(cl_bwd_apply_kernel<kGS, 1, false, true>, cl_grid(gm, nctas, gz), dim3(kT), st, use_pdl(), x, dz, nul, dx, gm, coef,
                         nul, nul, nul, nul, xd, dxd, coef_d)));
}

}
```

### dwt-domain-adaptation_b200/dwt_b200/csrc/norm_launch.h

```cpp
#pragma once
#include <stdint.h>

#include "dwt_common.cuh"

namespace dwt {

inline void bind_context() {
  thread_local bool bound = false;
  if (!bound) { cudaFree(nullptr); bound = true; }
}

bool small_supports(int GS);
void small_stats(const float* x, const Geom& gm, int vec, const FwdFin& fin, float* partial, int* counters,
                 cudaStream_t st);
void small_eval_prep(const Geom& gm, const FwdFin& fin, cudaStream_t st);
void small_apply(const float* x, float* y, const Geom& gm, int vec, int chunks, int epi, const float* mean,
                 const float* w, const float* gamma, const float* beta, const float* residual, cudaStream_t st);
void small_bwd_reduce(const float* x, const float* dout, const Geom& gm, int vec, const BwdFin& fin,
                      const float* beta, float* partial, int* counters, cudaStream_t st);
void small_bwd_prep(const Geom& gm, const BwdFin& fin, cudaStream_t st);
void small_bwd_apply(const float* x, const float* dout, float* dx, const Geom& gm, int vec, int chunks, int epi,
                     const float* coef, const float* mean, const float* w, const float* gamma, const float* beta,
                     cudaStream_t st);

int tiled_smem_bytes(int GS);
int tiled_init();
void tiled_stats(const float* x, const Geom& gm, int vec, const FwdFin& fin, float* partial, int* counters,
                 cudaStream_t st);
void tiled_eval_prep(const Geom& gm, const FwdFin& fin, cudaStream_t st);
void tiled_apply(const float* x, float* y, const Geom& gm, int vec, int chunks, const float* mean, const float* w,
                 cudaStream_t st);
void tiled_bwd_reduce(const float* x, const float* dout, const Geom& gm, int vec, const BwdFin& fin, float* partial,
                      int* counters, cudaStream_t st);
void tiled_bwd_prep(const Geom& gm, const BwdFin& fin, cudaStream_t st);
void tiled_bwd_apply(const float* x, const float* dout, float* dx, const Geom& gm, int vec, int chunks,
                     const float* coef, cudaStream_t st);

int tc_init();
bool tc_supports(const Geom& gm, int vec);
int tc_superblocks(const Geom& gm);
int tc_stats(const float* x, const Geom& gm, int nchunks, float* shift, float* partial, cudaStream_t st);
int tc_bwd_reduce(const float* x, const float* dout, const Geom& gm, int nchunks, const float* save_mean,
                  float* partial, cudaStream_t st);

int dense_init();
void dense_partial_reduce(const float* partial, int nchunks, int problems, float* gram, cudaStream_t st);
void dense_fwd_factor(const float* gram, const float* shift, const Geom& gm, const FwdFin& fin, cudaStream_t st);
void dense_bwd_coef(const float* rgram, const Geom& gm, const BwdFin& fin, float* dybar, cudaStream_t st);

int tc_apply_init();
int tc_apply(const float* x, float* y, const Geom& gm, int nctas, const float* save_mean, const float* save_w,
             cudaStream_t st);
int tc_bwd_apply(const float* x, const float* dout, float* dx, const Geom& gm, int nctas, const float* coef,
                 const float* save_mean, const float* dybar, cudaStream_t st);

bool cl_supports(int C, int GS);
int cl_fwd_width(int C, int GS);
int cl_bwd_width(int C, int GS);
void cl_stats(const float* x, const Geom& gm, int nctas, int gz, float* partial, float* shift, cudaStream_t st);
void cl_fwd_finalize(const float* partial, int nrows, const float* shift, const Geom& gm, const FwdFin& fin, cudaStream_t st,
                     const FwdFin* fin2 = nullptr, size_t pstride = 0, size_t sstride = 0);
void cl_apply(const float* x, float* y, const Geom& gm, int nctas, int gz, int epi, const float* mean, const float* w,
              const float* gamma, const float* beta, const float* residual, uint8_t* mask, cudaStream_t st);
void cl_bwd_reduce(const float* x, const float* dout, const float* dout2, const Geom& gm, int nctas, int gz, int epi, const float* mean, const float* w,
                   const float* gamma, const float* beta, const uint8_t* mask, float* dz, float* partial, cudaStream_t st);
void cl_bwd_finalize(const float* partial, int nrows, const Geom& gm, const BwdFin& fin, cudaStream_t st,
                     const BwdFin* fin2 = nullptr, size_t pstride = 0);
void cl_bwd_apply(const float* x, const float* dout, const float* dout2, float* dx, const Geom& gm, int nctas, int gz, int epi, const float* coef,
                  const float* mean, const float* w, const float* gamma, const float* beta, cudaStream_t st);
void cl_tail2_apply(const float* x, const float* xd, float* y, const Geom& gm, int nctas, int gz, const float* mean, const float* w,
                    const float* gamma, const float* beta, const float* mean_d, const float* w_d, const float* gamma_d,
                    const float* beta_d, uint8_t* mask, cudaStream_t st);
void cl_tail2_bwd_reduce(const float* x, const float* xd, const float* dout, const float* dout2, const Geom& gm, int nctas, int gz,
                         const float* mean, const float* mean_d, const uint8_t* mask, float* dz, float* partial, size_t pstride,
                         cudaStream_t st);
void cl_tail2_bwd_apply(const float* x, const float* xd, const float* dz, float* dx, float* dxd, const Geom& gm, int nctas, int gz,
                        const float* coef, const float* coef_d, cudaStream_t st);

void maxpool_fwd_launch(const float* x, float* y, uint8_t* idx, int N, int H, int W, int C, int OH, int OW, int k, int s, int p,
                        cudaStream_t st);
void maxpool_bwd_launch(const float* dy, const uint8_t* idx, float* dx, int N, int H, int W, int C, int OH, int OW, int k, int s,
                        int p, cudaStream_t st);

void augment_pair_launch(const uint8_t* images, int B, int SH, int SW, int CR, const int* crop_plain, const int* crop_aug,
                         const uint8_t* flip, const float* affine, const float* mean, const float* stdv,
                         float* out_plain, float* out_aug, int nhwc, cudaStream_t st);
void head_loss_launch(const float* logits, const long long* labels, int B, int K, float lambda, float* losses,
                      float* grad, int* status, cudaStream_t st);
void mec_launch(const float* x, const float* y, int N, int K, float* loss, float* gx, float* gy, cudaStream_t st);

}
```

### dwt-domain-adaptation_b200/dwt_b200/csrc/pool.cu

```cuda
#include "dwt_common.cuh"
#include "norm_launch.h"

namespace dwt {
namespace {

struct PoolGeom {
  int N, H, W, C4, OH, OW, k, s, p, c4shift;
};

template <int K, int S, int P>
__device__ __forceinline__ PoolGeom fixed(PoolGeom g) {
  if constexpr (K > 0) { g.k = K; g.s = S; g.p = P; }
  return g;
}

__device__ __forceinline__ bool takes(float v, float best) { return (v > best) || (v != v); }

template <int K, int S, int P, bool POW2>
__global__ void __launch_bounds__(256) maxpool_fwd_kernel(const float* __restrict__ x, float* __restrict__ y,
                                                          uint8_t* __restrict__ idx, const PoolGeom g0) {
  const PoolGeom g = fixed<K, S, P>(g0);
  const int n = blockIdx.x / g.OH, oh = blockIdx.x - n * g.OH;
  const int h0 = oh * g.s - g.p;
  const float4* xn = reinterpret_cast<const float4*>(x) + (size_t)n * g.H * g.W * g.C4;
  const size_t obase = ((size_t)n * g.OH + oh) * g.OW * g.C4;
  for (int t = threadIdx.x; t < g.OW * g.C4; t += blockDim.x) {
    const int ow = POW2 ? (t >> g.c4shift) : t / g.C4, c4 = t - ow * g.C4;
    const int w0 = ow * g.s - g.p;
    float best[4] = {-INFINITY, -INFINITY, -INFINITY, -INFINITY};
    unsigned bi[4] = {0u, 0u, 0u, 0u};
#pragma unroll
    for (int kh = 0; kh < g.k; ++kh) {
      const int h = h0 + kh;
      if (h < 0 || h >= g.H) continue;
      const float4* xr = xn + (size_t)h * g.W * g.C4 + c4;
#pragma unroll
      for (int kw = 0; kw < g.k; ++kw) {
        const int w = w0 + kw;
        if (w < 0 || w >= g.W) continue;
        const float4 v = __ldg(xr + (size_t)w * g.C4);
        const float e[4] = {v.x, v.y, v.z, v.w};
        const unsigned code = (unsigned)(kh * g.k + kw);
#pragma unroll
        for (int c = 0; c < 4; ++c)
          if (takes(e[c], best[c])) { best[c] = e[c]; bi[c] = code; }
      }
    }
    reinterpret_cast<float4*>(y)[obase + t] = make_float4(best[0], best[1], best[2], best[3]);
    reinterpret_cast<uint32_t*>(idx)[obase + t] = bi[0] | (bi[1] << 8) | (bi[2] << 16) | (bi[3] << 24);
  }
}

template <int K, int S, int P, bool POW2>
__global__ void __launch_bounds__(256) maxpool_bwd_kernel(const float* __restrict__ dy, const uint8_t* __restrict__ idx,
                                                          float* __restrict__ dx, const PoolGeom g0) {
  const PoolGeom g = fixed<K, S, P>(g0);
  const int n = blockIdx.x / g.H, h = blockIdx.x - n * g.H;
  int oh0 = h + g.p - g.k + 1;
  oh0 = oh0 <= 0 ? 0 : (oh0 + g.s - 1) / g.s;
  int oh1 = (h + g.p) / g.s;
  if (oh1 > g.OH - 1) oh1 = g.OH - 1;
  const float4* dyn = reinterpret_cast<const float4*>(dy) + (size_t)n * g.OH * g.OW * g.C4;
  const uint32_t* ixn = reinterpret_cast<const uint32_t*>(idx) + (size_t)n * g.OH * g.OW * g.C4;
  float4* dxr = reinterpret_cast<float4*>(dx) + ((size_t)n * g.H + h) * g.W * g.C4;
  for (int t = threadIdx.x; t < g.W * g.C4; t += blockDim.x) {
    const int w = POW2 ? (t >> g.c4shift) : t / g.C4, c4 = t - w * g.C4;
    int ow0 = w + g.p - g.k + 1;
    ow0 = ow0 <= 0 ? 0 : (ow0 + g.s - 1) / g.s;
    int ow1 = (w + g.p) / g.s;
    if (ow1 > g.OW - 1) ow1 = g.OW - 1;
    float acc[4] = {0.f, 0.f, 0.f, 0.f};
    for (int oh = oh0; oh <= oh1; ++oh) {
      const unsigned kh = (unsigned)(h - (oh * g.s - g.p));
      for (int ow = ow0; ow <= ow1; ++ow) {
        const unsigned code = kh * g.k + (unsigned)(w - (ow * g.s - g.p));
        const size_t o = ((size_t)oh * g.OW + ow) * g.C4 + c4;
        const uint32_t m = __ldg(ixn + o);
        const bool h0 = (m & 0xFFu) == code, h1 = ((m >> 8) & 0xFFu) == code, h2 = ((m >> 16) & 0xFFu) == code, h3 = (m >> 24) == code;
        if (h0 || h1 || h2 || h3) {
          const float4 gq = __ldg(dyn + o);
          if (h0) acc[0] += gq.x;
          if (h1) acc[1] += gq.y;
          if (h2) acc[2] += gq.z;
          if (h3) acc[3] += gq.w;
        }
      }
    }
    dxr[t] = make_float4(acc[0], acc[1], acc[2], acc[3]);
  }
}

__global__ void __launch_bounds__(256) maxpool_fwd_3s2_kernel(const float* __restrict__ x, float* __restrict__ y,
                                                              uint8_t* __restrict__ idx, const PoolGeom g) {
  const int OH2 = g.OH >> 1, OW2 = g.OW >> 1;
  const int n = blockIdx.y / OH2, a = blockIdx.y - n * OH2;
  const int i = blockIdx.x * blockDim.x + threadIdx.x;
  if (i >= OW2 * g.C4) return;
  const int b = i >> g.c4shift, c4 = i & (g.C4 - 1);
  const float4* xn = reinterpret_cast<const float4*>(x) + (size_t)n * g.H * g.W * g.C4 + c4;
  float best[2][2][4];
  unsigned bi[2][2][4];
#pragma unroll
  for (int oa = 0; oa < 2; ++oa)
#pragma unroll
    for (int ob = 0; ob < 2; ++ob)
#pragma unroll
      for (int c = 0; c < 4; ++c) { best[oa][ob][c] = -INFINITY; bi[oa][ob][c] = 0u; }
  const int h0 = 4 * a - 1, w0 = 4 * b - 1;
#pragma unroll
  for (int r = 0; r < 5; ++r) {
    const int h = h0 + r;
    if (h < 0 || h >= g.H) continue;
    float4 row[5];
    bool in[5];
#pragma unroll
    for (int cc = 0; cc < 5; ++cc) {
      const int w = w0 + cc;
      in[cc] = w >= 0 && w < g.W;
      row[cc] = in[cc] ? __ldg(xn + ((size_t)h * g.W + w) * g.C4) : make_float4(0.f, 0.f, 0.f, 0.f);
    }
#pragma unroll
    for (int oa = 0; oa < 2; ++oa) {
      const int kh = r - 2 * oa;
      if (kh < 0 || kh > 2) continue;
#pragma unroll
      for (int ob = 0; ob < 2; ++ob)
#pragma unroll
        for (int kw = 0; kw < 3; ++kw) {
          const int cc = 2 * ob + kw;
          if (!in[cc]) continue;
          const float e[4] = {row[cc].x, row[cc].y, row[cc].z, row[cc].w};
          const unsigned code = (unsigned)(kh * 3 + kw);
#pragma unroll
          for (int c = 0; c < 4; ++c)
            if (takes(e[c], best[oa][ob][c])) { best[oa][ob][c] = e[c]; bi[oa][ob][c] = code; }
        }
    }
  }
#pragma unroll
  for (int oa = 0; oa < 2; ++oa)
#pragma unroll
    for (int ob = 0; ob < 2; ++ob) {
      const size_t o = (((size_t)n * g.OH + 2 * a + oa) * g.OW + 2 * b + ob) * g.C4 + c4;
      reinterpret_cast<float4*>(y)[o] = make_float4(best[oa][ob][0], best[oa][ob][1], best[oa][ob][2], best[oa][ob][3]);
      reinterpret_cast<uint32_t*>(idx)[o] = bi[oa][ob][0] | (bi[oa][ob][1] << 8) | (bi[oa][ob][2] << 16) | (bi[oa][ob][3] << 24);
    }
}

__device__ __forceinline__ void take(float4& acc, const float4& gq, uint32_t m, unsigned code) {
  if ((m & 0xFFu) == code) acc.x += gq.x;
  if (((m >> 8) & 0xFFu) == code) acc.y += gq.y;
  if (((m >> 16) & 0xFFu) == code) acc.z += gq.z;
  if ((m >> 24) == code) acc.w += gq.w;
}

__global__ void __launch_bounds__(256) maxpool_bwd_3s2_kernel(const float* __restrict__ dy, const uint8_t* __restrict__ idx,
                                                              float* __restrict__ dx, const PoolGeom g) {
  const int H2 = g.H >> 1, W2 = g.W >> 1;
  const int n = blockIdx.y / H2, k = blockIdx.y - n * H2;
  const int i = blockIdx.x * blockDim.x + threadIdx.x;
  if (i >= W2 * g.C4) return;
  const int j = i >> g.c4shift, c4 = i & (g.C4 - 1);
  const float4* dyn = reinterpret_cast<const float4*>(dy) + (size_t)n * g.OH * g.OW * g.C4;
  const uint32_t* ixn = reinterpret_cast<const uint32_t*>(idx) + (size_t)n * g.OH * g.OW * g.C4;
  uint32_t m[2][2];
  float4 gq[2][2];
#pragma unroll
  for (int a = 0; a < 2; ++a)
#pragma unroll
    for (int b = 0; b < 2; ++b) {
      const bool ok = (k + a < g.OH) && (j + b < g.OW);
      const size_t o = ((size_t)(k + a) * g.OW + (j + b)) * g.C4 + c4;
      m[a][b] = ok ? __ldg(ixn + o) : 0xFFFFFFFFu;
      gq[a][b] = ok ? __ldg(dyn + o) : make_float4(0.f, 0.f, 0.f, 0.f);
    }
  float4 o00 = make_float4(0.f, 0.f, 0.f, 0.f), o01 = o00, o10 = o00, o11 = o00;
  take(o00, gq[0][0], m[0][0], 4u);
  take(o01, gq[0][0], m[0][0], 5u); take(o01, gq[0][1], m[0][1], 3u);
  take(o10, gq[0][0], m[0][0], 7u); take(o10, gq[1][0], m[1][0], 1u);
  take(o11, gq[0][0], m[0][0], 8u); take(o11, gq[0][1], m[0][1], 6u); take(o11, gq[1][0], m[1][0], 2u); take(o11, gq[1][1], m[1][1], 0u);
  float4* r0 = reinterpret_cast<float4*>(dx) + (((size_t)n * g.H + 2 * k) * g.W + 2 * j) * g.C4 + c4;
  float4* r1 = r0 + (size_t)g.W * g.C4;
  r0[0] = o00; r0[g.C4] = o01;
  r1[0] = o10; r1[g.C4] = o11;
}

}

namespace {
int pow2_shift(int v) {
  int sh = 0;
  while ((1 << sh) < v) ++sh;
  return (1 << sh) == v ? sh : -1;
}
}

void maxpool_fwd_launch(const float* x, float* y, uint8_t* idx, int N, int H, int W, int C, int OH, int OW, int k, int s, int p,
                        cudaStream_t st) {
  const int sh = pow2_shift(C / 4);
  const PoolGeom g{N, H, W, C / 4, OH, OW, k, s, p, sh < 0 ? 0 : sh};
  if (k == 3 && s == 2 && p == 1 && sh >= 0 && H % 4 == 0 && W % 4 == 0 && (long long)N * (OH / 2) <= 65535) {
    const int items = (OW / 2) * (C / 4), threads = items >= 256 ? 256 : ((items + 31) / 32) * 32;
    maxpool_fwd_3s2_kernel<<<dim3((items + threads - 1) / threads, N * (OH / 2)), threads, 0, st>>>(x, y, idx, g);
  } else if (k == 3 && s == 2 && p == 1 && sh >= 0) maxpool_fwd_kernel<3, 2, 1, true><<<N * OH, 256, 0, st>>>(x, y, idx, g);
  else maxpool_fwd_kernel<0, 0, 0, false><<<N * OH, 256, 0, st>>>(x, y, idx, g);
}

void maxpool_bwd_launch(const float* dy, const uint8_t* idx, float* dx, int N, int H, int W, int C, int OH, int OW, int k, int s,
                        int p, cudaStream_t st) {
  const int sh = pow2_shift(C / 4);
  const PoolGeom g{N, H, W, C / 4, OH, OW, k, s, p, sh < 0 ? 0 : sh};
  if (k == 3 && s == 2 && p == 1 && sh >= 0 && H % 2 == 0 && W % 2 == 0 && (long long)N * (H / 2) <= 65535) {
    const int items = (W / 2) * (C / 4), threads = items >= 256 ? 256 : ((items + 31) / 32) * 32;
    maxpool_bwd_3s2_kernel<<<dim3((items + threads - 1) / threads, N * (H / 2)), threads, 0, st>>>(dy, idx, dx, g);
  } else if (k == 3 && s == 2 && p == 1 && sh >= 0) maxpool_bwd_kernel<3, 2, 1, true><<<N * H, 256, 0, st>>>(dy, idx, dx, g);
  else maxpool_bwd_kernel<0, 0, 0, false><<<N * H, 256, 0, st>>>(dy, idx, dx, g);
}

}
```

### dwt-domain-adaptation_b200/dwt_b200/functional.py

```python
from __future__ import annotations

import torch

from . import _native as nv


def _dense(x: torch.Tensor, group_size: int):
    n, c = x.shape[0], x.shape[1]
    hw = 1
    for s in x.shape[2:]:
        hw *= s
    nhwc = (x.dim() == 4 and not x.is_contiguous() and x.is_contiguous(memory_format=torch.channels_last)
            and nv.channels_last_supported(c, group_size))
    if not nhwc and not x.is_contiguous():
        x = x.contiguous()
    return x, n, c, hw, nhwc


def _check_param(name, t, numel):
    if t is None:
        return
    if t.numel() != numel:
        raise ValueError(f"{name} has {t.numel()} elements, expected {numel}")
    if not t.is_contiguous():
        raise ValueError(f"{name} must be contiguous (it is written / read through a raw pointer)")


class _NormFunction(torch.autograd.Function):

    @staticmethod
    def forward(ctx, x, gamma, beta, residual, kind, group_size, n_domains, mode, eps, momentum, update_running,
                running, relu):
        lib = nv.lib()
        gs = group_size if kind == "whiten" else 1
        x, n_all, c, hw, nhwc = _dense(x, gs)
        layout = nv.LAYOUT_NHWC if nhwc else 0
        if n_all % n_domains != 0:
            raise ValueError(f"batch of {n_all} does not split into {n_domains} domains")
        n = n_all // n_domains
        dev = nv.require_cuda(x, gamma, beta, residual, *[t for pair in running for t in pair])
        for d, (rm_t, rv_t) in enumerate(running):
            _check_param(f"running mean of domain {d}", rm_t, c)
            _check_param(f"running second moment of domain {d}", rv_t, c * gs)
        _check_param("gamma / weight", gamma, c)
        _check_param("beta / bias", beta, c)
        epi = nv.EPI_NONE
        if residual is not None:
            if gamma is None or not relu or residual.shape != x.shape:
                raise ValueError("a fused residual needs gamma/beta, relu=True and a tensor shaped like x")
            residual = residual.contiguous(memory_format=torch.channels_last) if nhwc else residual.contiguous()
        if gamma is not None:
            epi = nv.EPI_AFFINE | (nv.EPI_RELU if relu else 0) | (nv.EPI_RESIDUAL if residual is not None else 0)
            gamma_c, beta_c = gamma.detach().reshape(-1).contiguous(), beta.detach().reshape(-1).contiguous()
        else:
            gamma_c = beta_c = None
        y = torch.empty_like(x)
        mask = torch.empty(x.numel() // 4, dtype=torch.uint8, device=dev) if (residual is not None and nhwc) else None
        save_mean = torch.empty(n_domains, c, dtype=torch.float32, device=dev)
        save_w = torch.empty(n_domains, c // gs, gs, gs, dtype=torch.float32, device=dev)
        ws = nv.workspace(dev, n, c, hw, gs, n_domains)
        need_running = (mode == nv.MODE_EVAL) or update_running
        rm = nv.ptr_array([p[0] for p in running]) if need_running else None
        rv = nv.ptr_array([p[1] for p in running]) if need_running else None
        with torch.cuda.device(dev):
            if kind == "whiten":
                rc = lib.dwt_whiten_fwd(nv.ptr(x), nv.ptr(y), n, c, hw, gs, n_domains, mode | layout, eps, momentum,
                                        int(update_running), rm, rv, nv.ptr(gamma_c), nv.ptr(beta_c), nv.ptr(residual),
                                        nv.ptr(mask), epi, nv.ptr(save_mean), nv.ptr(save_w), nv.ptr(ws), ws.numel(),
                                        nv.stream_ptr(dev))
            else:
                rc = lib.dwt_bn_fwd(nv.ptr(x), nv.ptr(y), n, c, hw, n_domains, mode | layout, eps, momentum,
                                    int(update_running), rm, rv, nv.ptr(gamma_c), nv.ptr(beta_c), nv.ptr(residual),
                                    nv.ptr(mask), epi, nv.ptr(save_mean), nv.ptr(save_w), nv.ptr(ws), ws.numel(),
                                    nv.stream_ptr(dev))
        nv.check(rc)
        nv.poll_status(dev)
        if update_running and mode == nv.MODE_TRAIN:
            seen = set()
            for pair in running:
                for buf in pair:
                    if buf is not None and id(buf) not in seen:
                        seen.add(id(buf))
                        torch.autograd.graph.increment_version(buf)
        ctx.residual_mode = None
        if mask is not None:
            ctx.save_for_backward(x, save_mean, save_w, gamma_c, beta_c, mask)
            ctx.residual_mode = "mask"
        elif residual is not None:
            ctx.save_for_backward(x, save_mean, save_w, gamma_c, beta_c, y)
            epi = nv.EPI_AFFINE
            ctx.residual_mode = "aten"
        else:
            ctx.save_for_backward(x, save_mean, save_w, gamma_c, beta_c)
        ctx.cfg = (kind, gs, n_domains, mode | layout, eps, epi, n, c, hw, None if gamma is None else gamma.shape)
        return y

    @staticmethod
    def backward(ctx, dout):
        lib = nv.lib()
        mask = None
        if ctx.residual_mode == "mask":
            x, save_mean, save_w, gamma_c, beta_c, mask = ctx.saved_tensors
        elif ctx.residual_mode == "aten":
            x, save_mean, save_w, gamma_c, beta_c, out = ctx.saved_tensors
            extra = ctx.__dict__.pop("_dwt_extra_grad", None)
            if extra is not None:
                dout = dout + extra
            dout = torch.ops.aten.threshold_backward(dout, out, 0)
        else:
            x, save_mean, save_w, gamma_c, beta_c = ctx.saved_tensors
        kind, gs, n_domains, mode, eps, epi, n, c, hw, gshape = ctx.cfg
        dout2 = ctx.__dict__.pop("_dwt_extra_grad", None)
        if dout2 is not None and not ((mode & nv.LAYOUT_NHWC) and dout2.shape == dout.shape and dout2.dtype == torch.float32
                                      and dout2.is_contiguous(memory_format=torch.channels_last)):
            dout, dout2 = dout + dout2, None
        dout = dout.contiguous(memory_format=torch.channels_last) if (mode & nv.LAYOUT_NHWC) else dout.contiguous()
        dev = nv.require_cuda(dout)
        dx = torch.empty_like(x)
        want_affine = gamma_c is not None and (ctx.needs_input_grad[1] or ctx.needs_input_grad[2])
        d_res = None
        if ctx.residual_mode == "mask":
            d_res = torch.empty_like(x)
        elif ctx.residual_mode == "aten" and ctx.needs_input_grad[3]:
            d_res = dout
        dgamma = torch.empty(c, dtype=torch.float32, device=dev) if want_affine else None
        dbeta = torch.empty(c, dtype=torch.float32, device=dev) if want_affine else None
        ws = nv.workspace(dev, n, c, hw, gs, n_domains)
        with torch.cuda.device(dev):
            if kind == "whiten":
                rc = lib.dwt_whiten_bwd(nv.ptr(x), nv.ptr(dout), nv.ptr(dout2), nv.ptr(dx), n, c, hw, gs, n_domains, mode, eps,
                                        nv.ptr(save_mean), nv.ptr(save_w), nv.ptr(gamma_c), nv.ptr(beta_c), nv.ptr(mask),
                                        nv.ptr(d_res) if mask is not None else None, epi,
                                        nv.ptr(dgamma), nv.ptr(dbeta), nv.ptr(ws), ws.numel(), nv.stream_ptr(dev))
            else:
                rc = lib.dwt_bn_bwd(nv.ptr(x), nv.ptr(dout), nv.ptr(dout2), nv.ptr(dx), n, c, hw, n_domains, mode,
                                    nv.ptr(save_mean), nv.ptr(save_w), nv.ptr(gamma_c), nv.ptr(beta_c), nv.ptr(mask),
                                    nv.ptr(d_res) if mask is not None else None, epi,
                                    nv.ptr(dgamma), nv.ptr(dbeta), nv.ptr(ws), ws.numel(), nv.stream_ptr(dev))
        nv.check(rc)
        if want_affine:
            dgamma, dbeta = dgamma.view(gshape), dbeta.view(gshape)
        return (dx, dgamma, dbeta, d_res if ctx.needs_input_grad[3] else None) + (None,) * 9


class _TailPairFunction(torch.autograd.Function):

    @staticmethod
    def forward(ctx, x, xd, gamma, beta, gamma_d, beta_d, kind, group_size, n_domains, sites):
        lib = nv.lib()
        gs = group_size if kind == "whiten" else 1
        if not (x.dim() == 4 and x.shape == xd.shape and _dense(x, gs)[4] and _dense(xd, gs)[4]):
            raise ValueError("the two-site tail takes two channels-last tensors of one shape with a channels-last build")
        if x.shape[0] % n_domains != 0:
            raise ValueError(f"batch of {x.shape[0]} does not split into {n_domains} domains")
        n_all, c = x.shape[0], x.shape[1]
        hw = x.shape[2] * x.shape[3]
        n = n_all // n_domains
        dev = nv.require_cuda(x, xd, gamma, beta, gamma_d, beta_d, *[t for run, *_ in sites for pair in run for t in pair])
        params = [(gamma, beta), (gamma_d, beta_d)]
        c_sites = (nv.TailSite * 2)()
        keep = []
        saved = []
        for k, (inp, (g, b), (running, eps, momentum, update)) in enumerate(zip((x, xd), params, sites)):
            for d, (rm_t, rv_t) in enumerate(running):
                _check_param(f"running mean of domain {d}", rm_t, c)
                _check_param(f"running second moment of domain {d}", rv_t, c * gs)
            _check_param("gamma / weight", g, c)
            _check_param("beta / bias", b, c)
            g_c, b_c = g.detach().reshape(-1).contiguous(), b.detach().reshape(-1).contiguous()
            save_mean = torch.empty(n_domains, c, dtype=torch.float32, device=dev)
            save_w = torch.empty(n_domains, c // gs, gs, gs, dtype=torch.float32, device=dev)
            rm = nv.ptr_array([pr[0] for pr in running]) if update else None
            rv = nv.ptr_array([pr[1] for pr in running]) if update else None
            c_sites[k] = nv.TailSite(inp.data_ptr(), eps, momentum, int(update), rm, rv, g_c.data_ptr(), b_c.data_ptr(),
                                     save_mean.data_ptr(), save_w.data_ptr(), None, None, None)
            keep += [g_c, b_c, rm, rv]
            saved += [save_mean, save_w, g_c]
        y = torch.empty_like(x)
        mask = torch.empty(x.numel() // 4, dtype=torch.uint8, device=dev)
        ws = nv.workspace(dev, n, c, hw, gs, n_domains)
        nv_kind = nv.KIND_WHITEN if kind == "whiten" else nv.KIND_BN
        with torch.cuda.device(dev):
            rc = lib.dwt_tail2_fwd(nv_kind, c_sites, nv.ptr(y), nv.ptr(mask), n, c, hw, gs, n_domains, nv.ptr(ws), ws.numel(),
                                   nv.stream_ptr(dev))
        nv.check(rc)
        nv.poll_status(dev)
        seen = set()
        for running, _, _, update in sites:
            for buf in (t for pair in running for t in pair) if update else ():
                if id(buf) not in seen:
                    seen.add(id(buf))
                    torch.autograd.graph.increment_version(buf)
        ctx.save_for_backward(x, xd, mask, *saved)
        ctx.cfg = (nv_kind, gs, n_domains, n, c, hw, [s[1] for s in sites], gamma.shape, gamma_d.shape)
        return y

    @staticmethod
    def backward(ctx, dout):
        lib = nv.lib()
        x, xd, mask, mean0, w0, g0, mean1, w1, g1 = ctx.saved_tensors
        nv_kind, gs, n_domains, n, c, hw, eps, gshape, gshape_d = ctx.cfg
        dout2 = ctx.__dict__.pop("_dwt_extra_grad", None)
        if dout2 is not None and not (dout2.shape == dout.shape and dout2.dtype == torch.float32
                                      and dout2.is_contiguous(memory_format=torch.channels_last)):
            dout, dout2 = dout + dout2, None
        dout = dout.contiguous(memory_format=torch.channels_last)
        dev = nv.require_cuda(dout)
        dz = torch.empty_like(x)
        dx, dxd = torch.empty_like(x), torch.empty_like(xd)
        grads = [torch.empty(2, c, dtype=torch.float32, device=dev) for _ in range(2)]
        c_sites = (nv.TailSite * 2)()
        for k, (inp, mean, w, g, d_in, gr) in enumerate(zip((x, xd), (mean0, mean1), (w0, w1), (g0, g1), (dx, dxd), grads)):
            c_sites[k] = nv.TailSite(inp.data_ptr(), eps[k], 0.0, 0, None, None, g.data_ptr(), g.data_ptr(), mean.data_ptr(),
                                     w.data_ptr(), d_in.data_ptr(), gr[0].data_ptr(), gr[1].data_ptr())
        ws = nv.workspace(dev, n, c, hw, gs, n_domains)
        with torch.cuda.device(dev):
            rc = lib.dwt_tail2_bwd(nv_kind, c_sites, nv.ptr(dout), nv.ptr(dout2), nv.ptr(mask), nv.ptr(dz), n, c, hw, gs, n_domains,
                                   nv.ptr(ws), ws.numel(), nv.stream_ptr(dev))
        nv.check(rc)
        return (dx, dxd, grads[0][0].view(gshape), grads[0][1].view(gshape), grads[1][0].view(gshape_d),
                grads[1][1].view(gshape_d)) + (None,) * 4


def tail_pair(x, xd, gamma, beta, gamma_d, beta_d, *, kind, group_size, n_domains, sites):
    return _TailPairFunction.apply(x, xd, gamma, beta, gamma_d, beta_d, kind, group_size, n_domains,
                                   [(r, float(e), float(m), bool(u)) for r, e, m, u in sites])


class _ForkForSum(torch.autograd.Function):

    @staticmethod
    def forward(ctx, y):
        ctx.producer = y.grad_fn
        return y.view_as(y), y.view_as(y)

    @staticmethod
    def backward(ctx, ga, gb):
        producer, ctx.producer = ctx.producer, None
        if ga is None or gb is None:
            return ga if gb is None else gb
        if producer is None or "_dwt_extra_grad" in producer.__dict__:
            return ga + gb
        producer.__dict__["_dwt_extra_grad"] = gb
        return ga


def fork_for_sum(y):
    fn = getattr(y, "grad_fn", None)
    if not torch.is_grad_enabled() or fn is None or not isinstance(fn, (_NormFunction._backward_cls, _TailPairFunction._backward_cls)):
        return y, y
    return _ForkForSum.apply(y)


def norm(x, gamma, beta, *, kind, group_size, n_domains, training_stats, eps, momentum, update_running,
         running, relu=False, residual=None):
    mode = nv.MODE_TRAIN if training_stats else nv.MODE_EVAL
    return _NormFunction.apply(x, gamma, beta, residual, kind, group_size, n_domains, mode, float(eps),
                               float(momentum), bool(update_running), running, bool(relu))


class _MecFunction(torch.autograd.Function):
    @staticmethod
    def forward(ctx, x, y):
        lib = nv.lib()
        if x.dim() != 2 or x.shape != y.shape:
            raise ValueError(f"expected two [N, K] logit tensors, got {tuple(x.shape)} and {tuple(y.shape)}")
        x, y = x.contiguous(), y.contiguous()
        dev = nv.require_cuda(x, y)
        loss = torch.empty((), dtype=torch.float32, device=dev)
        gx, gy = torch.empty_like(x), torch.empty_like(y)
        with torch.cuda.device(dev):
            rc = lib.dwt_mec_fwd_bwd(nv.ptr(x), nv.ptr(y), x.shape[0], x.shape[1], nv.ptr(loss), nv.ptr(gx),
                                     nv.ptr(gy), nv.stream_ptr(dev))
        nv.check(rc)
        ctx.save_for_backward(gx, gy)
        return loss

    @staticmethod
    def backward(ctx, g):
        gx, gy = ctx.saved_tensors
        return g * gx, g * gy


def mec_loss(x, y):
    return _MecFunction.apply(x, y)


class _HeadLossFunction(torch.autograd.Function):
    @staticmethod
    def forward(ctx, logits, labels, lam):
        lib = nv.lib()
        if logits.dim() != 2 or logits.shape[0] % 3 != 0 or labels.dim() != 1 or labels.shape[0] * 3 != logits.shape[0]:
            raise ValueError(f"expected logits [3B, K] and labels [B], got {tuple(logits.shape)} and {tuple(labels.shape)}")
        logits = logits.contiguous()
        dev = nv.require_cuda(logits)
        if not labels.is_cuda or labels.dtype != torch.int64:
            raise nv.NativeError("labels must be an int64 CUDA tensor")
        labels = labels.contiguous()
        losses = torch.empty(3, dtype=torch.float32, device=dev)
        grad = torch.empty_like(logits)
        with torch.cuda.device(dev):
            rc = lib.dwt_head_loss_fwd_bwd(nv.ptr(logits), nv.ptr(labels), labels.shape[0], logits.shape[1], float(lam),
                                           nv.ptr(losses), nv.ptr(grad), nv.status_ptr(dev), nv.stream_ptr(dev))
        nv.check(rc)
        nv.poll_status(dev)
        ctx.save_for_backward(grad)
        ctx.mark_non_differentiable(losses)
        return losses[0], losses

    @staticmethod
    def backward(ctx, g, _unused):
        (grad,) = ctx.saved_tensors
        return g * grad, None, None


def head_loss(logits, labels, lambda_mec):
    return _HeadLossFunction.apply(logits, labels, lambda_mec)
```

### dwt-domain-adaptation_b200/dwt_b200/fused.py

```python
from __future__ import annotations

import torch
import torch.nn as nn

from . import _native as nv
from . import functional as F


class DomainTripleNorm(nn.Module):
    def __init__(self, kind, num_features, group_size=4, n_domains=3):
        super().__init__()
        if kind not in ("whiten", "bn"):
            raise ValueError("kind must be 'whiten' or 'bn'")
        self.kind, self.num_features, self.n_domains = kind, num_features, n_domains
        self.group_size = min(num_features, group_size) if kind == "whiten" else 1
        self.kernel_epilogue = self.group_size in (1, 2, 4)

    def forward(self, x, domain_modules, gamma, beta, relu=False, residual=None, replicated=False, count_batches=True):
        mods = list(domain_modules)
        if len(mods) != self.n_domains:
            raise ValueError(f"expected {self.n_domains} domain modules")
        if x.dim() != 4:
            raise ValueError('expected 4D input (got {}D input)'.format(x.dim()))
        if replicated:
            return self._forward_replicated(x, mods, gamma, beta, relu, residual, count_batches)
        running, eps, momentum, update = self._running_args(mods, count_batches)
        if not self.kernel_epilogue:
            y = F.norm(x, None, None, kind=self.kind, group_size=self.group_size, n_domains=self.n_domains,
                       training_stats=True, eps=eps, momentum=momentum, update_running=update, running=running)
            return self._tensor_epilogue(y, gamma, beta, relu, residual)
        return F.norm(x, gamma, beta, kind=self.kind, group_size=self.group_size, n_domains=self.n_domains,
                      training_stats=True, eps=eps, momentum=momentum, update_running=update,
                      running=running, relu=relu, residual=residual)

    def _running_args(self, mods, count_batches):
        m0 = mods[0]
        if self.kind == "whiten":
            running = [(m.running_mean, m.running_variance) for m in mods]
            eps, momentum = m0.eps, m0.momentum
        else:
            if count_batches:
                counters = [m.num_batches_tracked for m in mods if m.training and m.track_running_stats]
                if counters:
                    torch._foreach_add_(counters, 1)
            running = [(m.running_mean, m.running_var) for m in mods]
            eps = m0.eps
            momentum = m0.momentum if m0.momentum is not None else 1.0 / m0.num_batches_tracked.item()
        return running, eps, momentum, m0.training and m0.track_running_stats

    def forward_with_downsample(self, x, domain_modules, gamma, beta, xd, down, down_modules, down_gamma, down_beta,
                                count_batches=True):
        mods, down_mods = list(domain_modules), list(down_modules)
        pair = (self.kernel_epilogue and down.kernel_epilogue and self.kind == down.kind
                and self.group_size == down.group_size and self.n_domains == down.n_domains
                and len(mods) == len(down_mods) == self.n_domains and x.dim() == 4 and x.shape == xd.shape
                and all(t.is_contiguous(memory_format=torch.channels_last) and not t.is_contiguous() for t in (x, xd))
                and nv.channels_last_supported(x.shape[1], self.group_size))
        if not pair:
            identity = down(xd, down_mods, down_gamma, down_beta, relu=False, count_batches=count_batches)
            return self(x, mods, gamma, beta, True, residual=identity, count_batches=count_batches)
        down_args = down._running_args(down_mods, count_batches)
        site_args = self._running_args(mods, count_batches)
        return F.tail_pair(x, xd, gamma, beta, down_gamma, down_beta, kind=self.kind, group_size=self.group_size,
                           n_domains=self.n_domains, sites=(site_args, down_args))

    @staticmethod
    def _tensor_epilogue(y, gamma, beta, relu, residual):
        if residual is not None and not relu:
            raise ValueError("a fused residual needs relu=True")
        if gamma is not None:
            y = y * gamma + beta
        if residual is not None:
            y = y + residual
        return torch.relu(y) if relu else y

    def _forward_replicated(self, x, mods, gamma, beta, relu, residual, count_batches=True):
        second = "running_variance" if self.kind == "whiten" else "running_var"
        keep = {}
        for m in mods:
            if not (m.training and m.track_running_stats):
                continue
            if self.kind == "bn":
                if count_batches:
                    m.num_batches_tracked += 1
                f = m.momentum if m.momentum is not None else 1.0 / m.num_batches_tracked.item()
            else:
                f = m.momentum
            rm, rv = m.running_mean, getattr(m, second)
            key = (rm.data_ptr(), rv.data_ptr())
            prod, _ = keep.get(key, (1.0, None))
            keep[key] = (prod * (1.0 - f), (rm, rv))
        means = {k[0] for k in keep}
        seconds = {k[1] for k in keep}
        if len(means) != len(keep) or len(seconds) != len(keep):
            raise ValueError("replicated statistics need each running_mean paired with one second-moment buffer")
        m0 = mods[0]
        common = dict(kind=self.kind, group_size=self.group_size, n_domains=1, training_stats=True, eps=m0.eps)
        if self.kernel_epilogue:
            common.update(relu=relu, residual=residual)
            g_arg, b_arg = gamma, beta
        else:
            g_arg = b_arg = None
        if not keep:
            out = F.norm(x, g_arg, b_arg, momentum=0.0, update_running=False,
                         running=[(m0.running_mean, getattr(m0, second))], **common)
        else:
            out = None
            for prod, pair in keep.values():
                y = F.norm(x, g_arg, b_arg, momentum=1.0 - prod, update_running=True, running=[pair], **common)
                out = y if out is None else out
        return out if self.kernel_epilogue else self._tensor_epilogue(out, gamma, beta, relu, residual)
```

### harness/resnet50_dwt.py

```python
from __future__ import annotations

import torch
import torch.nn as nn

_STAGES = ((64, 3, 1), (128, 4, 2), (256, 6, 2), (512, 3, 2))
_DOMAINS = ("s", "t", "t_aug")
EXPANSION = 4


_REPLICATED = [False]
_BATCHED_COUNTERS = [False]


class WhitenScaleShift(nn.Module):

    def __init__(self, layers, planes, group_size, running_mean, running_variance,
                 track_running_stats=True, affine=True):
        super().__init__()
        self.planes, self.group_size, self.affine = planes, group_size, affine
        self.wh = layers.WTransform2d(planes, group_size, running_m=running_mean,
                                      running_var=running_variance,
                                      track_running_stats=track_running_stats)
        if affine:
            self.gamma = nn.Parameter(torch.ones(planes, 1, 1))
            self.beta = nn.Parameter(torch.zeros(planes, 1, 1))

    def forward(self, x):
        y = self.wh(x)
        return y * self.gamma + self.beta if self.affine else y


class _SiteOwner(nn.Module):

    def _add_site(self, layers, tag, key, planes, whiten, group_size, stats, site_mode):
        pre, post = ("downsample_", "") if tag == "downsample" else ("", tag)
        names = [f"{pre}bn{d}{post}" if d != "t_aug" else f"{pre}bnt{post}_aug" for d in _DOMAINS]
        if whiten:
            rm, rv = stats[key + ".wh.running_mean"], stats[key + ".wh.running_variance"]
            gamma, beta = stats[key + ".gamma"], stats[key + ".beta"]
            mods = [WhitenScaleShift(layers, planes, group_size, rm, rv, affine=False) for _ in names]
        else:
            rm, rv = stats[key + ".running_mean"], stats[key + ".running_var"]
            gamma, beta = stats[key + ".weight"].view(-1, 1, 1), stats[key + ".bias"].view(-1, 1, 1)
            mods = [layers.BatchNorm2d(num_features=planes, running_m=rm, running_v=rv, affine=False)
                    for _ in names]
        for n, m in zip(names, mods):
            setattr(self, n, m)
        gname = f"{pre}gamma{post}" if pre == "" else "downsample_gamma"
        bname = f"{pre}beta{post}" if pre == "" else "downsample_beta"
        setattr(self, gname, nn.Parameter(gamma))
        setattr(self, bname, nn.Parameter(beta))
        if not hasattr(self, "_sites"):
            self._sites = {}
        self._sites[tag] = (names, gname, bname, whiten)
        if site_mode == "fused":
            object.__setattr__(self, f"_fused_{tag}", layers.DomainTripleNorm(
                kind="whiten" if whiten else "bn", num_features=planes,
                group_size=group_size if whiten else 1))

    def _site(self, tag, x, relu, residual=None):
        names, gname, bname, whiten = self._sites[tag]
        gamma, beta = getattr(self, gname), getattr(self, bname)
        if residual is not None:
            fused = getattr(self, f"_fused_{tag}", None) if self.training else None
            if fused is not None:
                mods = [getattr(self, n) for n in names]
                return fused(x, [m.wh if whiten else m for m in mods], gamma, beta, True, residual=residual,
                             replicated=_REPLICATED[0], count_batches=not _BATCHED_COUNTERS[0])
            return torch.relu_(self._site(tag, x, relu=False) + residual)
        if self.training:
            fused = getattr(self, f"_fused_{tag}", None)
            mods = [getattr(self, n) for n in names]
            if fused is not None:
                return fused(x, [m.wh if whiten else m for m in mods], gamma, beta, relu, replicated=_REPLICATED[0],
                             count_batches=not _BATCHED_COUNTERS[0])
            if _REPLICATED[0]:
                raise RuntimeError("replicated statistics collection needs site_mode='fused'")
            parts = torch.split(x, x.shape[0] // 3, dim=0)
            s, t, a = (m(p) for m, p in zip(mods, parts))
            out = torch.cat((s, torch.cat((t, a), dim=0)), dim=0) * gamma + beta
        else:
            out = getattr(self, names[1])(x) * gamma + beta
        return torch.relu_(out) if relu else out


class Bottleneck(_SiteOwner):
    def __init__(self, layers, inplanes, planes, layer, sub_layer, stats, group_size, stride,
                 downsample, site_mode):
        super().__init__()
        whiten = layer == 1
        key = f"layer{layer}.{sub_layer}"
        self.conv1 = nn.Conv2d(inplanes, planes, 1, bias=False)
        self._add_site(layers, "1", key + ".bn1", planes, whiten, group_size, stats, site_mode)
        self.conv2 = nn.Conv2d(planes, planes, 3, stride=stride, padding=1, bias=False)
        self._add_site(layers, "2", key + ".bn2", planes, whiten, group_size, stats, site_mode)
        self.conv3 = nn.Conv2d(planes, planes * EXPANSION, 1, bias=False)
        self._add_site(layers, "3", key + ".bn3", planes * EXPANSION, whiten, group_size, stats, site_mode)
        self.downsample = downsample
        if downsample is not None:
            self._add_site(layers, "downsample", f"layer{layer}.0.downsample_bn", planes * EXPANSION,
                           whiten, group_size, stats, site_mode)
        object.__setattr__(self, "_fork", getattr(layers, "fork_for_sum", None) if site_mode == "fused" else None)

    def forward(self, x):
        xa, xb = self._fork(x) if (self._fork is not None and self.training) else (x, x)
        out = self._site("1", self.conv1(xa), relu=True)
        out = self._site("2", self.conv2(out), relu=True)
        if self.downsample is None:
            return self._site("3", self.conv3(out), relu=True, residual=xb)
        tail = getattr(self, "_fused_3", None) if (self.training and not _REPLICATED[0]) else None
        if tail is None:
            identity = self._site("downsample", self.downsample(xb), relu=False)
            return self._site("3", self.conv3(out), relu=True, residual=identity)
        xd = self.downsample(xb)
        names, gname, bname, whiten = self._sites["3"]
        dnames, dgname, dbname, _ = self._sites["downsample"]
        unwrap = (lambda m: m.wh) if whiten else (lambda m: m)
        return tail.forward_with_downsample(
            self.conv3(out), [unwrap(getattr(self, n)) for n in names], getattr(self, gname), getattr(self, bname),
            xd, self._fused_downsample, [unwrap(getattr(self, n)) for n in dnames], getattr(self, dgname),
            getattr(self, dbname), count_batches=not _BATCHED_COUNTERS[0])


class ResNet50DWT(_SiteOwner):
    def __init__(self, layers, state_dict, num_classes=65, group_size=4, site_mode="modules", stem_pad=0, stem_nchw=False,
                 stem_s2d=False):
        super().__init__()
        self.stem_s2d = stem_s2d
        self.stem_nchw = stem_nchw
        self.stem_pad = stem_pad
        if site_mode not in ("modules", "fused"):
            raise ValueError("site_mode must be 'modules' or 'fused'")
        stats = {k: v for k, v in state_dict.items() if "bn" in k or "downsample" in k}
        self.site_mode = site_mode
        self.conv1 = nn.Conv2d(3, 64, 7, stride=2, padding=3, bias=False)
        self._add_site(layers, "1", "bn1", 64, True, group_size, stats, site_mode)
        self.maxpool = nn.MaxPool2d(3, stride=2, padding=1)
        inplanes = 64
        for li, (planes, blocks, stride) in enumerate(_STAGES, start=1):
            seq = []
            for b in range(blocks):
                down = None
                if b == 0 and (stride != 1 or inplanes != planes * EXPANSION):
                    down = nn.Sequential(nn.Conv2d(inplanes, planes * EXPANSION, 1, stride=stride, bias=False))
                seq.append(Bottleneck(layers, inplanes, planes, li, b, stats, 4, stride if b == 0 else 1,
                                      down, site_mode))
                inplanes = planes * EXPANSION
            setattr(self, f"layer{li}", nn.Sequential(*seq))
        self.avgpool = nn.AdaptiveAvgPool2d((1, 1))
        self.fc_out = nn.Linear(512 * EXPANSION, num_classes)
        for m in self.modules():
            if isinstance(m, nn.Conv2d):
                nn.init.kaiming_normal_(m.weight, mode="fan_out", nonlinearity="relu")

    def _stem_s2d(self, x):
        n, c, h, w = x.shape
        if h % 2 or w % 2:
            return self.conv1(x)
        cl = x.is_contiguous(memory_format=torch.channels_last) and not x.is_contiguous()
        xp = torch.nn.functional.pad(x, (3, 3, 3, 3))
        hp, wp = (h + 6) // 2, (w + 6) // 2
        wt = torch.nn.functional.pad(self.conv1.weight, (0, 1, 0, 1))
        o = wt.shape[0]
        if cl:
            xs = xp.view(n, c, hp, 2, wp, 2).permute(0, 2, 4, 1, 3, 5).reshape(n, hp, wp, 4 * c).permute(0, 3, 1, 2)
            w4 = wt.view(o, c, 4, 2, 4, 2).permute(0, 2, 4, 1, 3, 5).reshape(o, 4, 4, 4 * c).permute(0, 3, 1, 2)
        else:
            xs = xp.view(n, c, hp, 2, wp, 2).permute(0, 1, 3, 5, 2, 4).reshape(n, 4 * c, hp, wp)
            w4 = wt.view(o, c, 4, 2, 4, 2).permute(0, 1, 3, 5, 2, 4).reshape(o, 4 * c, 4, 4)
        return torch.nn.functional.conv2d(xs, w4)

    def _stem(self, x):
        if self.stem_s2d:
            return self._stem_s2d(x)
        if self.stem_nchw:
            return self.conv1(x.contiguous()).contiguous(memory_format=torch.channels_last)
        if not self.stem_pad or x.shape[1] >= self.stem_pad:
            return self.conv1(x)
        extra = self.stem_pad - x.shape[1]
        fmt = torch.channels_last if (x.is_contiguous(memory_format=torch.channels_last) and not x.is_contiguous()) \
            else torch.contiguous_format
        xp = torch.zeros((x.shape[0], self.stem_pad) + tuple(x.shape[2:]), dtype=x.dtype, device=x.device).contiguous(memory_format=fmt)
        xp[:, :x.shape[1]] = x
        w = torch.nn.functional.pad(self.conv1.weight, (0, 0, 0, 0, 0, extra))
        if fmt == torch.channels_last:
            w = w.contiguous(memory_format=torch.channels_last)
        c = self.conv1
        return torch.nn.functional.conv2d(xp, w, None, c.stride, c.padding, c.dilation, c.groups)

    def _bump_counters(self):
        cs = getattr(self, "_bn_counters", None)
        if cs is None:
            cs = [m.num_batches_tracked for m in self.modules()
                  if hasattr(m, "num_batches_tracked") and m.num_batches_tracked is not None and getattr(m, "track_running_stats", False)]
            object.__setattr__(self, "_bn_counters", cs)
        if cs:
            torch._foreach_add_(cs, 1)

    def forward(self, x):
        batched = self.training and self.site_mode == "fused"
        if batched:
            self._bump_counters()
        _BATCHED_COUNTERS[0] = batched
        try:
            x = self.maxpool(self._site("1", self._stem(x), relu=True))
            x = self.layer4(self.layer3(self.layer2(self.layer1(x))))
        finally:
            _BATCHED_COUNTERS[0] = False
        return self.fc_out(torch.flatten(self.avgpool(x), 1))


def build_resnet50_dwt(state_dict, layers, site_mode="modules", num_classes=65, channels_last=False, stem_pad=0,
                       stem_nchw=False, stem_s2d=False):
    model = ResNet50DWT(layers, state_dict, num_classes=num_classes, site_mode=site_mode, stem_pad=stem_pad,
                        stem_nchw=stem_nchw and channels_last, stem_s2d=stem_s2d)
    model.load_state_dict(state_dict, strict=False)
    if channels_last and hasattr(layers, "MaxPool2d"):
        model.maxpool = layers.MaxPool2d(3, stride=2, padding=1)
    if channels_last:
        for m in model.modules():
            if isinstance(m, nn.Conv2d) and not (model.stem_nchw and m is model.conv1):
                m.weight.data = m.weight.data.contiguous(memory_format=torch.channels_last)
    return model


def collect_stats(model, batches, passes=1, replicated=True):
    was_training = model.training
    model.train(True)
    out = None
    try:
        with torch.no_grad():
            for _ in range(passes):
                for data in batches:
                    if replicated:
                        _REPLICATED[0] = True
                        out = model(data)
                    else:
                        out = model(torch.cat((data, data, data), dim=0))
    finally:
        _REPLICATED[0] = False
        model.train(was_training)
    return out
```

### include/dwt_b200.h

```cpp
#ifndef DWT_B200_H_
#define DWT_B200_H_

#include <stddef.h>
#include <stdint.h>

#ifdef __cplusplus
extern "C" {
#endif

#define DWT_B200_ABI_VERSION 6
#define DWT_MAX_DOMAINS 4
#define DWT_MAX_GROUP_SIZE 64

#define DWT_OK 0
#define DWT_E_INVALID (-1)
#define DWT_E_WORKSPACE (-2)
#define DWT_E_LAUNCH (-3)
#define DWT_E_UNSUPPORTED (-4)

#define DWT_MODE_TRAIN 0
#define DWT_MODE_EVAL 1

#define DWT_LAYOUT_NHWC 0x100

#define DWT_EPI_NONE 0
#define DWT_EPI_AFFINE 1
#define DWT_EPI_RELU 2
#define DWT_EPI_RESIDUAL 4

typedef struct CUstream_st *dwt_stream_t;

#if defined(__GNUC__)
#define DWT_API __attribute__((visibility("default")))
#else
#define DWT_API
#endif

DWT_API int dwt_abi_version(void);
DWT_API const char *dwt_last_error(void);

DWT_API size_t dwt_workspace_bytes(int64_t N, int64_t C, int64_t HW, int group_size, int n_domains);

#define DWT_STATUS_NOT_PD 1
#define DWT_STATUS_BAD_LABEL 2

DWT_API int dwt_whiten_fwd(const float *x, float *y, int64_t N, int64_t C, int64_t HW, int group_size,
                   int n_domains, int mode, float eps, float momentum, int update_running,
                   float *const *running_mean, float *const *running_cov, const float *gamma,
                   const float *beta, const float *residual, uint8_t *relu_mask, int epilogue, float *save_mean,
                   float *save_w, void *workspace, size_t workspace_bytes, dwt_stream_t stream);

DWT_API int dwt_whiten_bwd(const float *x, const float *dout, const float *dout2, float *dx, int64_t N, int64_t C, int64_t HW,
                   int group_size, int n_domains, int mode, float eps, const float *save_mean,
                   const float *save_w, const float *gamma, const float *beta, const uint8_t *relu_mask,
                   float *dresidual, int epilogue, float *dgamma, float *dbeta, void *workspace,
                   size_t workspace_bytes, dwt_stream_t stream);

DWT_API int dwt_bn_fwd(const float *x, float *y, int64_t N, int64_t C, int64_t HW, int n_domains, int mode,
               float eps, float factor, int update_running, float *const *running_mean,
               float *const *running_var, const float *weight, const float *bias, const float *residual,
               uint8_t *relu_mask, int epilogue, float *save_mean, float *save_invstd, void *workspace,
               size_t workspace_bytes, dwt_stream_t stream);

DWT_API int dwt_bn_bwd(const float *x, const float *dout, const float *dout2, float *dx, int64_t N, int64_t C, int64_t HW,
               int n_domains, int mode, const float *save_mean, const float *save_invstd,
               const float *weight, const float *bias, const uint8_t *relu_mask, float *dresidual, int epilogue,
               float *dweight, float *dbias, void *workspace, size_t workspace_bytes, dwt_stream_t stream);

#define DWT_KIND_WHITEN 0
#define DWT_KIND_BN 1
typedef struct {
  const float *x;
  float eps, momentum;
  int update_running;
  float *const *running_mean;
  float *const *running_cov;
  const float *gamma, *beta;
  float *save_mean, *save_w;
  float *dx;
  float *dgamma, *dbeta;
} dwt_tail_site;

DWT_API int dwt_tail2_fwd(int kind, const dwt_tail_site *sites, float *y, uint8_t *relu_mask, int64_t N, int64_t C,
                  int64_t HW, int group_size, int n_domains, void *workspace, size_t workspace_bytes,
                  dwt_stream_t stream);
DWT_API int dwt_tail2_bwd(int kind, const dwt_tail_site *sites, const float *dout, const float *dout2,
                  const uint8_t *relu_mask, float *dz, int64_t N, int64_t C, int64_t HW, int group_size,
                  int n_domains, void *workspace, size_t workspace_bytes, dwt_stream_t stream);

DWT_API int dwt_mec_fwd_bwd(const float *x, const float *y, int64_t N, int64_t K, float *loss, float *gx,
                    float *gy, dwt_stream_t stream);

DWT_API int dwt_head_loss_fwd_bwd(const float *logits, const int64_t *labels, int64_t B, int64_t K, float lambda,
                          float *losses, float *grad, int *status, dwt_stream_t stream);

DWT_API int dwt_augment_pair(const uint8_t *images, int64_t B, int src_h, int src_w, int crop, const int32_t *crop_plain,
                     const int32_t *crop_aug, const uint8_t *flip, const float *affine, const float *mean,
                     const float *stdv, float *out_plain, float *out_aug, int layout, dwt_stream_t stream);

DWT_API int dwt_maxpool_fwd(const float *x, float *y, uint8_t *argmax, int64_t N, int64_t H, int64_t W, int64_t C,
                    int kernel, int stride, int padding, dwt_stream_t stream);
DWT_API int dwt_maxpool_bwd(const float *dy, const uint8_t *argmax, float *dx, int64_t N, int64_t H, int64_t W, int64_t C,
                    int kernel, int stride, int padding, dwt_stream_t stream);

typedef struct {
  char name[48];
  int64_t launches;
  double ms;
  double bytes;
} dwt_profile_entry;

DWT_API int64_t dwt_launch_count(void);
DWT_API void dwt_profile_begin(void);
DWT_API int dwt_profile_end(dwt_profile_entry *out, int max_entries);

#ifdef __cplusplus
}
#endif
#endif
```

Measured before the change: 2882.

## Fuse stem whitening apply with 3x3 max-pool in forward and backward

Adds a pooled-site path that computes stem whitening/BN statistics, then applies the normalisation, affine, ReLU and 3x3/2 max-pool in one kernel, writing only the pooled output and argmax codes. This removes the write and re-read of the full-resolution normalised activation. Backward runs the maxpool backward (which can now also fold in a second incoming gradient) straight into the site backward reduce and apply. The cost is recomputing the whitening for overlapping pool windows, plus a new stem path that only activates under training, channels-last layout and H/W divisible by 4.

```diff
diff --git a/dwt-domain-adaptation_b200/dwt_b200/_native.py b/dwt-domain-adaptation_b200/dwt_b200/_native.py
--- a/dwt-domain-adaptation_b200/dwt_b200/_native.py
+++ b/dwt-domain-adaptation_b200/dwt_b200/_native.py
@@ -9,7 +9,7 @@
 _HERE = os.path.dirname(os.path.abspath(__file__))
 LIB_PATH = os.environ.get("DWT_B200_LIB") or os.path.join(_HERE, "lib", "libdwt_b200.so")
 
-ABI_VERSION = 6
+ABI_VERSION = 7
 MAX_DOMAINS = 4
 MAX_GROUP_SIZE = 64
 MODE_TRAIN, MODE_EVAL = 0, 1
@@ -58,6 +58,14 @@
     "dwt_tail2_bwd": (ctypes.c_int, [ctypes.c_int, ctypes.POINTER(TailSite), _c_float_p, _c_float_p, ctypes.c_void_p,
                                      _c_float_p, ctypes.c_int64, ctypes.c_int64, ctypes.c_int64, ctypes.c_int, ctypes.c_int,
                                      ctypes.c_void_p, ctypes.c_size_t, ctypes.c_void_p]),
+    "dwt_site_pool_fwd": (ctypes.c_int, [ctypes.c_int, _c_float_p, _c_float_p, ctypes.c_void_p, ctypes.c_int64, ctypes.c_int64,
+                                         ctypes.c_int64, ctypes.c_int64, ctypes.c_int, ctypes.c_int, ctypes.c_float, ctypes.c_float,
+                                         ctypes.c_int, ctypes.POINTER(ctypes.c_void_p), ctypes.POINTER(ctypes.c_void_p), _c_float_p,
+                                         _c_float_p, _c_float_p, _c_float_p, ctypes.c_void_p, ctypes.c_size_t, ctypes.c_void_p]),
+    "dwt_site_pool_bwd": (ctypes.c_int, [ctypes.c_int, _c_float_p, _c_float_p, _c_float_p, ctypes.c_void_p, _c_float_p, _c_float_p, ctypes.c_int64,
+                                         ctypes.c_int64, ctypes.c_int64, ctypes.c_int64, ctypes.c_int, ctypes.c_int, ctypes.c_float,
+                                         _c_float_p, _c_float_p, _c_float_p, _c_float_p, _c_float_p, _c_float_p, ctypes.c_void_p,
+                                         ctypes.c_size_t, ctypes.c_void_p]),
     "dwt_mec_fwd_bwd": (ctypes.c_int, [_c_float_p, _c_float_p, ctypes.c_int64, ctypes.c_int64, _c_float_p,
                                        _c_float_p, _c_float_p, ctypes.c_void_p]),
     "dwt_head_loss_fwd_bwd": (ctypes.c_int, [_c_float_p, ctypes.c_void_p, ctypes.c_int64, ctypes.c_int64, ctypes.c_float,
diff --git a/dwt-domain-adaptation_b200/dwt_b200/csrc/api.cu b/dwt-domain-adaptation_b200/dwt_b200/csrc/api.cu
--- a/dwt-domain-adaptation_b200/dwt_b200/csrc/api.cu
+++ b/dwt-domain-adaptation_b200/dwt_b200/csrc/api.cu
@@ -586,6 +586,100 @@
   return check_launch("channels-last two-site backward apply kernel");
 }
 
+int site_pool_plan(Plan& p, dwt::PoolDims& pd, int kind, const float* x, const float* pooled, const uint8_t* argmax, int64_t N,
+                   int64_t C, int64_t H, int64_t W, int GS, int D) {
+  if (kind != DWT_KIND_WHITEN && kind != DWT_KIND_BN) return fail(DWT_E_INVALID, "bad kind %d", kind);
+  if (kind == DWT_KIND_BN && GS != 1) return fail(DWT_E_INVALID, "batch norm has group_size 1 (got %d)", GS);
+  if (H <= 0 || W <= 0 || H % 4 != 0 || W % 4 != 0)
+    return fail(DWT_E_UNSUPPORTED, "the pooled site is built for H and W multiples of 4 (got %lldx%lld)", (long long)H, (long long)W);
+  if (int rc = make_plan(p, K_STATS, K_APPLY, x, pooled, argmax, N, C, H * W, GS, D)) return rc;
+  if (!dwt::cl_supports((int)C, GS))
+    return fail(DWT_E_UNSUPPORTED, "the pooled site runs on the channels-last kernels: group_size 1, 2, 4 with C/4 a power of two (C=%lld gs=%d)",
+                (long long)C, GS);
+  if (!x || !pooled || !argmax) return fail(DWT_E_INVALID, "null pointer argument");
+  if ((((uintptr_t)x | (uintptr_t)pooled | (uintptr_t)argmax) % 16) != 0) return fail(DWT_E_INVALID, "channels-last tensors must be 16-byte aligned");
+  if ((int64_t)D * N * (H / 2) > 65535) return fail(DWT_E_UNSUPPORTED, "n_domains * N * H / 2 = %lld exceeds one grid dimension", (long long)D * N * (H / 2));
+  pd = dwt::PoolDims{(int)H, (int)W, (int)H / 2, (int)W / 2};
+  return DWT_OK;
+}
+
+int site_pool_workspace(Workspace& w, void* ws, size_t ws_bytes, int64_t C, int GS, int D) {
+  if (!ws) return fail(DWT_E_INVALID, "null pointer argument");
+  w = carve(ws, C, GS, D);
+  if (w.bytes > ws_bytes) return fail(DWT_E_WORKSPACE, "workspace too small: need %zu bytes, got %zu", w.bytes, ws_bytes);
+  if ((uintptr_t)ws % 256 != 0) return fail(DWT_E_WORKSPACE, "workspace must be 256-byte aligned");
+  return DWT_OK;
+}
+
+int site_pool_fwd(int kind, const float* x, float* y, uint8_t* argmax, int64_t N, int64_t C, int64_t H, int64_t W, int GS, int D,
+                  float eps, float momentum, int update_running, float* const* rmean, float* const* rcov, const float* gamma,
+                  const float* beta, float* save_mean, float* save_w, void* ws, size_t ws_bytes, cudaStream_t st) {
+  Plan p;
+  dwt::PoolDims pd;
+  if (int rc = site_pool_plan(p, pd, kind, x, y, argmax, N, C, H, W, GS, D)) return rc;
+  if (!gamma || !beta || !save_mean || !save_w) return fail(DWT_E_INVALID, "null pointer argument");
+  if (int rc = check_running(update_running != 0, rmean, rcov, D)) return rc;
+  Workspace w;
+  if (int rc = site_pool_workspace(w, ws, ws_bytes, C, GS, D)) return rc;
+  const SiteConst sc = site_const(kind, eps, N, H * W);
+  const dwt::FwdFin fin = make_fwd_fin(sc.a, sc.b, momentum, sc.unbias, update_running, update_running != 0, rmean, rcov, save_mean,
+                                       save_w, w, D);
+  const double E = 4.0 * (double)D * (double)N * (double)C * (double)(H * W);
+  const ClPlan cp = cl_plan(p.gm, 3, 3, 8, 8);
+  {
+    Launch l("cl_stats", &p.gm, E, st);
+    dwt::cl_stats(x, p.gm, cp.nred, cp.gz_red, w.partial, w.shift, st);
+  }
+  if (int rc = check_launch("channels-last statistics kernel")) return rc;
+  {
+    Launch l("cl_fwd_finalize", &p.gm, 0.0, st);
+    dwt::cl_fwd_finalize(w.partial, cp.nred, w.shift, p.gm, fin, st);
+  }
+  if (int rc = check_launch("channels-last finalize kernel")) return rc;
+  {
+    Launch l("cl_pool_apply", &p.gm, E + E / 4 + E / 16, st);
+    dwt::cl_pool_apply(x, y, reinterpret_cast<uint32_t*>(argmax), p.gm, pd, save_mean, save_w, gamma, beta, st);
+  }
+  return check_launch("pooled site apply kernel");
+}
+
+int site_pool_bwd(int kind, const float* x, const float* dy, const float* dy2, const uint8_t* argmax, float* dsite, float* dx,
+                  int64_t N, int64_t C, int64_t H, int64_t W, int GS, int D, float eps, const float* save_mean, const float* save_w,
+                  const float* gamma, const float* beta, float* dgamma, float* dbeta, void* ws, size_t ws_bytes, cudaStream_t st) {
+  Plan p;
+  dwt::PoolDims pd;
+  if (int rc = site_pool_plan(p, pd, kind, x, dy, argmax, N, C, H, W, GS, D)) return rc;
+  if (!dsite || !dx || !save_mean || !save_w || !gamma || !beta) return fail(DWT_E_INVALID, "null pointer argument");
+  if ((((uintptr_t)dsite | (uintptr_t)dx | (uintptr_t)dy2) % 16) != 0) return fail(DWT_E_INVALID, "channels-last tensors must be 16-byte aligned");
+  if ((dgamma == nullptr) != (dbeta == nullptr)) return fail(DWT_E_INVALID, "dgamma and dbeta go together");
+  Workspace w;
+  if (int rc = site_pool_workspace(w, ws, ws_bytes, C, GS, D)) return rc;
+  const int epi = DWT_EPI_AFFINE | DWT_EPI_RELU;
+  const dwt::BwdFin fin = make_bwd_fin(site_const(kind, eps, N, H * W).a, DWT_MODE_TRAIN, epi, save_mean, save_w, gamma, dgamma, dbeta, w);
+  const double E = 4.0 * (double)D * (double)N * (double)C * (double)(H * W), P = E / 4, I = E / 16;
+  {
+    Launch l("maxpool_bwd", nullptr, E + P + I + (dy2 ? P : 0.0), st);
+    dwt::maxpool_bwd_launch(dy, argmax, dsite, (int)(D * N), (int)H, (int)W, (int)C, pd.OH, pd.OW, 3, 2, 1, st, dy2);
+  }
+  if (int rc = check_launch("max-pool backward kernel")) return rc;
+  const ClPlan cp = cl_plan(p.gm, 2, 2, 4, 4);
+  {
+    Launch l("cl_bwd_reduce", &p.gm, 2.0 * E, st);
+    dwt::cl_bwd_reduce(x, dsite, nullptr, p.gm, cp.nred, cp.gz_red, epi, save_mean, save_w, gamma, beta, nullptr, nullptr, w.partial, st);
+  }
+  if (int rc = check_launch("channels-last backward reduction kernel")) return rc;
+  {
+    Launch l("cl_bwd_finalize", &p.gm, 0.0, st);
+    dwt::cl_bwd_finalize(w.partial, cp.nred, p.gm, fin, st);
+  }
+  if (int rc = check_launch("channels-last backward finalize kernel")) return rc;
+  {
+    Launch l("cl_bwd_apply", &p.gm, 3.0 * E, st);
+    dwt::cl_bwd_apply(x, dsite, nullptr, dx, p.gm, cp.new_, cp.gz_ew, epi, w.coef, save_mean, save_w, gamma, beta, st);
+  }
+  return check_launch("channels-last backward apply kernel");
+}
+
 }
 
 extern "C" {
@@ -651,6 +745,22 @@
                   dwt_stream_t stream) {
   return tail2_bwd(kind, sites, dout, dout2, relu_mask, dz, N, C, HW, group_size, n_domains, workspace, workspace_bytes,
                    (cudaStream_t)stream);
+}
+
+int dwt_site_pool_fwd(int kind, const float* x, float* y, uint8_t* argmax, int64_t N, int64_t C, int64_t H, int64_t W, int group_size,
+                      int n_domains, float eps, float momentum, int update_running, float* const* running_mean, float* const* running_cov,
+                      const float* gamma, const float* beta, float* save_mean, float* save_w, void* workspace, size_t workspace_bytes,
+                      dwt_stream_t stream) {
+  return site_pool_fwd(kind, x, y, argmax, N, C, H, W, group_size, n_domains, eps, momentum, update_running, running_mean, running_cov,
+                       gamma, beta, save_mean, save_w, workspace, workspace_bytes, (cudaStream_t)stream);
+}
+
+int dwt_site_pool_bwd(int kind, const float* x, const float* dy, const float* dy2, const uint8_t* argmax, float* dsite, float* dx,
+                      int64_t N, int64_t C, int64_t H, int64_t W, int group_size, int n_domains, float eps, const float* save_mean,
+                      const float* save_w, const float* gamma, const float* beta, float* dgamma, float* dbeta, void* workspace,
+                      size_t workspace_bytes, dwt_stream_t stream) {
+  return site_pool_bwd(kind, x, dy, dy2, argmax, dsite, dx, N, C, H, W, group_size, n_domains, eps, save_mean, save_w, gamma, beta, dgamma,
+                       dbeta, workspace, workspace_bytes, (cudaStream_t)stream);
 }
 
 int dwt_mec_fwd_bwd(const float* x, const float* y, int64_t N, int64_t K, float* loss, float* gx, float* gy,
diff --git a/dwt-domain-adaptation_b200/dwt_b200/csrc/norm_cl.cu b/dwt-domain-adaptation_b200/dwt_b200/csrc/norm_cl.cu
--- a/dwt-domain-adaptation_b200/dwt_b200/csrc/norm_cl.cu
+++ b/dwt-domain-adaptation_b200/dwt_b200/csrc/norm_cl.cu
@@ -2,6 +2,7 @@
 
 #include "dwt_common.cuh"
 #include "norm_launch.h"
+#include "pool_common.cuh"
 #include "small_algebra.cuh"
 
 namespace dwt {
@@ -325,6 +326,89 @@
       }
     });
   }
+}
+
+template <int GS>
+__global__ void __launch_bounds__(256) cl_pool_apply_kernel(const float* __restrict__ x, float* __restrict__ y, uint32_t* __restrict__ idx,
+                                                            const Geom gm, const PoolDims pd, const float* __restrict__ save_mean,
+                                                            const float* __restrict__ save_w, const float* __restrict__ gamma,
+                                                            const float* __restrict__ beta) {
+  using S = ClShape<GS>;
+  const int C4 = gm.C >> 2, OH2 = pd.OH >> 1;
+  const int n = blockIdx.y / OH2, a = blockIdx.y - n * OH2;
+  const int i = blockIdx.x * blockDim.x + threadIdx.x;
+  pdl_wait();
+  if (i >= (pd.OW >> 1) * C4) return;
+  const int b = i >> (__ffs(C4) - 1), q = i & (C4 - 1);
+  const int d = n / gm.N;
+  float Wp[S::NSUB][S::NM], bp[S::NSUB][GS];
+#pragma unroll
+  for (int s = 0; s < S::NSUB; ++s) {
+    const int g = q * S::NSUB + s;
+    load_forward_map<GS, DWT_EPI_AFFINE | DWT_EPI_RELU>(save_w + ((size_t)d * gm.G + g) * GS * GS, save_mean + (size_t)d * gm.C + g * GS,
+                                                        gamma + g * GS, beta + g * GS, Wp[s], bp[s]);
+  }
+  const float* xn = x + (size_t)n * gm.HW * gm.C + 4 * q;
+  float best[2][2][4];
+  unsigned bi[2][2][4];
+#pragma unroll
+  for (int oa = 0; oa < 2; ++oa)
+#pragma unroll
+    for (int ob = 0; ob < 2; ++ob)
+#pragma unroll
+      for (int c = 0; c < 4; ++c) { best[oa][ob][c] = -INFINITY; bi[oa][ob][c] = 0u; }
+  const int h0 = 4 * a - 1, w0 = 4 * b - 1;
+#pragma unroll
+  for (int r = 0; r < 5; ++r) {
+    const int h = h0 + r;
+    if (h < 0 || h >= pd.H) continue;
+    float4 v[5];
+    bool in[5];
+#pragma unroll
+    for (int cc = 0; cc < 5; ++cc) {
+      const int w = w0 + cc;
+      in[cc] = w >= 0 && w < pd.W;
+      v[cc] = in[cc] ? ldg4(xn + ((size_t)h * pd.W + w) * gm.C) : make_float4(0.f, 0.f, 0.f, 0.f);
+    }
+    float row[5][4];
+#pragma unroll
+    for (int cc = 0; cc < 5; ++cc) {
+      const float e[4] = {v[cc].x, v[cc].y, v[cc].z, v[cc].w};
+#pragma unroll
+      for (int s = 0; s < S::NSUB; ++s) {
+        float xi[GS], oi[GS];
+#pragma unroll
+        for (int c = 0; c < GS; ++c) xi[c] = e[s * GS + c];
+        apply_group<GS>(Wp[s], bp[s], xi, oi);
+#pragma unroll
+        for (int c = 0; c < GS; ++c) row[cc][s * GS + c] = fmaxf(oi[c], 0.f);
+      }
+    }
+#pragma unroll
+    for (int oa = 0; oa < 2; ++oa) {
+      const int kh = r - 2 * oa;
+      if (kh < 0 || kh > 2) continue;
+#pragma unroll
+      for (int ob = 0; ob < 2; ++ob)
+#pragma unroll
+        for (int kw = 0; kw < 3; ++kw) {
+          const int cc = 2 * ob + kw;
+          if (!in[cc]) continue;
+          const unsigned code = (unsigned)(kh * 3 + kw);
+#pragma unroll
+          for (int c = 0; c < 4; ++c)
+            if (takes(row[cc][c], best[oa][ob][c])) { best[oa][ob][c] = row[cc][c]; bi[oa][ob][c] = code; }
+        }
+    }
+  }
+#pragma unroll
+  for (int oa = 0; oa < 2; ++oa)
+#pragma unroll
+    for (int ob = 0; ob < 2; ++ob) {
+      const size_t o = (((size_t)n * pd.OH + 2 * a + oa) * pd.OW + 2 * b + ob) * C4 + q;
+      reinterpret_cast<float4*>(y)[o] = make_float4(best[oa][ob][0], best[oa][ob][1], best[oa][ob][2], best[oa][ob][3]);
+      idx[o] = pack_codes(bi[oa][ob]);
+    }
 }
 
 template <int GS>
@@ -717,4 +801,11 @@
                          nul, nul, nul, nul, xd, dxd, coef_d)));
 }
 
-}
+void cl_pool_apply(const float* x, float* y, uint32_t* argmax, const Geom& gm, const PoolDims& pd, const float* mean, const float* w,
+                   const float* gamma, const float* beta, cudaStream_t st) {
+  const int items = (pd.OW / 2) * (gm.C / 4), threads = items >= 256 ? 256 : ((items + 31) / 32) * 32;
+  const dim3 grid((items + threads - 1) / threads, gm.D * gm.N * (pd.OH / 2));
+  CL_GS(gm.GS, (launch_k(cl_pool_apply_kernel<kGS>, grid, dim3(threads), st, use_pdl(), x, y, argmax, gm, pd, mean, w, gamma, beta)));
+}
+
+}
diff --git a/dwt-domain-adaptation_b200/dwt_b200/csrc/norm_launch.h b/dwt-domain-adaptation_b200/dwt_b200/csrc/norm_launch.h
--- a/dwt-domain-adaptation_b200/dwt_b200/csrc/norm_launch.h
+++ b/dwt-domain-adaptation_b200/dwt_b200/csrc/norm_launch.h
@@ -76,11 +76,14 @@
                          cudaStream_t st);
 void cl_tail2_bwd_apply(const float* x, const float* xd, const float* dz, float* dx, float* dxd, const Geom& gm, int nctas, int gz,
                         const float* coef, const float* coef_d, cudaStream_t st);
+struct PoolDims { int H, W, OH, OW; };
+void cl_pool_apply(const float* x, float* y, uint32_t* argmax, const Geom& gm, const PoolDims& pd, const float* mean, const float* w,
+                   const float* gamma, const float* beta, cudaStream_t st);
 
 void maxpool_fwd_launch(const float* x, float* y, uint8_t* idx, int N, int H, int W, int C, int OH, int OW, int k, int s, int p,
                         cudaStream_t st);
 void maxpool_bwd_launch(const float* dy, const uint8_t* idx, float* dx, int N, int H, int W, int C, int OH, int OW, int k, int s,
-                        int p, cudaStream_t st);
+                        int p, cudaStream_t st, const float* dy2 = nullptr);
 
 void augment_pair_launch(const uint8_t* images, int B, int SH, int SW, int CR, const int* crop_plain, const int* crop_aug,
                          const uint8_t* flip, const float* affine, const float* mean, const float* stdv,
diff --git a/dwt-domain-adaptation_b200/dwt_b200/csrc/pool.cu b/dwt-domain-adaptation_b200/dwt_b200/csrc/pool.cu
--- a/dwt-domain-adaptation_b200/dwt_b200/csrc/pool.cu
+++ b/dwt-domain-adaptation_b200/dwt_b200/csrc/pool.cu
@@ -1,5 +1,6 @@
 #include "dwt_common.cuh"
 #include "norm_launch.h"
+#include "pool_common.cuh"
 
 namespace dwt {
 namespace {
@@ -13,8 +14,6 @@
   if constexpr (K > 0) { g.k = K; g.s = S; g.p = P; }
   return g;
 }
-
-__device__ __forceinline__ bool takes(float v, float best) { return (v > best) || (v != v); }
 
 template <int K, int S, int P, bool POW2>
 __global__ void __launch_bounds__(256) maxpool_fwd_kernel(const float* __restrict__ x, float* __restrict__ y,
@@ -47,7 +46,7 @@
       }
     }
     reinterpret_cast<float4*>(y)[obase + t] = make_float4(best[0], best[1], best[2], best[3]);
-    reinterpret_cast<uint32_t*>(idx)[obase + t] = bi[0] | (bi[1] << 8) | (bi[2] << 16) | (bi[3] << 24);
+    reinterpret_cast<uint32_t*>(idx)[obase + t] = pack_codes(bi);
   }
 }
 
@@ -143,25 +142,20 @@
     for (int ob = 0; ob < 2; ++ob) {
       const size_t o = (((size_t)n * g.OH + 2 * a + oa) * g.OW + 2 * b + ob) * g.C4 + c4;
       reinterpret_cast<float4*>(y)[o] = make_float4(best[oa][ob][0], best[oa][ob][1], best[oa][ob][2], best[oa][ob][3]);
-      reinterpret_cast<uint32_t*>(idx)[o] = bi[oa][ob][0] | (bi[oa][ob][1] << 8) | (bi[oa][ob][2] << 16) | (bi[oa][ob][3] << 24);
-    }
-}
-
-__device__ __forceinline__ void take(float4& acc, const float4& gq, uint32_t m, unsigned code) {
-  if ((m & 0xFFu) == code) acc.x += gq.x;
-  if (((m >> 8) & 0xFFu) == code) acc.y += gq.y;
-  if (((m >> 16) & 0xFFu) == code) acc.z += gq.z;
-  if ((m >> 24) == code) acc.w += gq.w;
-}
-
-__global__ void __launch_bounds__(256) maxpool_bwd_3s2_kernel(const float* __restrict__ dy, const uint8_t* __restrict__ idx,
-                                                              float* __restrict__ dx, const PoolGeom g) {
+      reinterpret_cast<uint32_t*>(idx)[o] = pack_codes(bi[oa][ob]);
+    }
+}
+
+template <bool D2>
+__global__ void __launch_bounds__(256) maxpool_bwd_3s2_kernel(const float* __restrict__ dy, const float* __restrict__ dy2,
+                                                              const uint8_t* __restrict__ idx, float* __restrict__ dx, const PoolGeom g) {
   const int H2 = g.H >> 1, W2 = g.W >> 1;
   const int n = blockIdx.y / H2, k = blockIdx.y - n * H2;
   const int i = blockIdx.x * blockDim.x + threadIdx.x;
   if (i >= W2 * g.C4) return;
   const int j = i >> g.c4shift, c4 = i & (g.C4 - 1);
   const float4* dyn = reinterpret_cast<const float4*>(dy) + (size_t)n * g.OH * g.OW * g.C4;
+  const float4* dy2n = D2 ? reinterpret_cast<const float4*>(dy2) + (size_t)n * g.OH * g.OW * g.C4 : nullptr;
   const uint32_t* ixn = reinterpret_cast<const uint32_t*>(idx) + (size_t)n * g.OH * g.OW * g.C4;
   uint32_t m[2][2];
   float4 gq[2][2];
@@ -173,6 +167,10 @@
       const size_t o = ((size_t)(k + a) * g.OW + (j + b)) * g.C4 + c4;
       m[a][b] = ok ? __ldg(ixn + o) : 0xFFFFFFFFu;
       gq[a][b] = ok ? __ldg(dyn + o) : make_float4(0.f, 0.f, 0.f, 0.f);
+      if constexpr (D2) {
+        const float4 q2 = ok ? __ldg(dy2n + o) : make_float4(0.f, 0.f, 0.f, 0.f);
+        gq[a][b].x += q2.x; gq[a][b].y += q2.y; gq[a][b].z += q2.z; gq[a][b].w += q2.w;
+      }
     }
   float4 o00 = make_float4(0.f, 0.f, 0.f, 0.f), o01 = o00, o10 = o00, o11 = o00;
   take(o00, gq[0][0], m[0][0], 4u);
@@ -207,12 +205,14 @@
 }
 
 void maxpool_bwd_launch(const float* dy, const uint8_t* idx, float* dx, int N, int H, int W, int C, int OH, int OW, int k, int s,
-                        int p, cudaStream_t st) {
+                        int p, cudaStream_t st, const float* dy2) {
   const int sh = pow2_shift(C / 4);
   const PoolGeom g{N, H, W, C / 4, OH, OW, k, s, p, sh < 0 ? 0 : sh};
   if (k == 3 && s == 2 && p == 1 && sh >= 0 && H % 2 == 0 && W % 2 == 0 && (long long)N * (H / 2) <= 65535) {
     const int items = (W / 2) * (C / 4), threads = items >= 256 ? 256 : ((items + 31) / 32) * 32;
-    maxpool_bwd_3s2_kernel<<<dim3((items + threads - 1) / threads, N * (H / 2)), threads, 0, st>>>(dy, idx, dx, g);
+    const dim3 grid((items + threads - 1) / threads, N * (H / 2));
+    if (dy2) maxpool_bwd_3s2_kernel<true><<<grid, threads, 0, st>>>(dy, dy2, idx, dx, g);
+    else maxpool_bwd_3s2_kernel<false><<<grid, threads, 0, st>>>(dy, nullptr, idx, dx, g);
   } else if (k == 3 && s == 2 && p == 1 && sh >= 0) maxpool_bwd_kernel<3, 2, 1, true><<<N * H, 256, 0, st>>>(dy, idx, dx, g);
   else maxpool_bwd_kernel<0, 0, 0, false><<<N * H, 256, 0, st>>>(dy, idx, dx, g);
 }
diff --git a/dwt-domain-adaptation_b200/dwt_b200/csrc/pool_common.cuh b/dwt-domain-adaptation_b200/dwt_b200/csrc/pool_common.cuh
--- /dev/null
+++ b/dwt-domain-adaptation_b200/dwt_b200/csrc/pool_common.cuh
@@ -0,0 +1,19 @@
+#pragma once
+#include <stdint.h>
+
+namespace dwt {
+
+__device__ __forceinline__ bool takes(float v, float best) { return (v > best) || (v != v); }
+
+__device__ __forceinline__ uint32_t pack_codes(const unsigned (&bi)[4]) {
+  return bi[0] | (bi[1] << 8) | (bi[2] << 16) | (bi[3] << 24);
+}
+
+__device__ __forceinline__ void take(float4& acc, const float4& gq, uint32_t m, unsigned code) {
+  if ((m & 0xFFu) == code) acc.x += gq.x;
+  if (((m >> 8) & 0xFFu) == code) acc.y += gq.y;
+  if (((m >> 16) & 0xFFu) == code) acc.z += gq.z;
+  if ((m >> 24) == code) acc.w += gq.w;
+}
+
+}
diff --git a/dwt-domain-adaptation_b200/dwt_b200/functional.py b/dwt-domain-adaptation_b200/dwt_b200/functional.py
--- a/dwt-domain-adaptation_b200/dwt_b200/functional.py
+++ b/dwt-domain-adaptation_b200/dwt_b200/functional.py
@@ -227,6 +227,82 @@
                                    [(r, float(e), float(m), bool(u)) for r, e, m, u in sites])
 
 
+class _SitePoolFunction(torch.autograd.Function):
+
+    @staticmethod
+    def forward(ctx, x, gamma, beta, kind, group_size, n_domains, site):
+        lib = nv.lib()
+        gs = group_size if kind == "whiten" else 1
+        running, eps, momentum, update = site
+        if not (x.dim() == 4 and _dense(x, gs)[4] and x.shape[2] % 4 == 0 and x.shape[3] % 4 == 0):
+            raise ValueError("the pooled site takes a channels-last tensor with a channels-last build and H, W multiples of 4")
+        n_all, c, h, w = x.shape
+        if n_all % n_domains != 0:
+            raise ValueError(f"batch of {n_all} does not split into {n_domains} domains")
+        n = n_all // n_domains
+        dev = nv.require_cuda(x, gamma, beta, *[t for pair in running for t in pair])
+        for d, (rm_t, rv_t) in enumerate(running):
+            _check_param(f"running mean of domain {d}", rm_t, c)
+            _check_param(f"running second moment of domain {d}", rv_t, c * gs)
+        _check_param("gamma / weight", gamma, c)
+        _check_param("beta / bias", beta, c)
+        gamma_c, beta_c = gamma.detach().reshape(-1).contiguous(), beta.detach().reshape(-1).contiguous()
+        y = torch.empty((n_all, c, h // 2, w // 2), dtype=torch.float32, device=dev, memory_format=torch.channels_last)
+        argmax = torch.empty(y.numel(), dtype=torch.uint8, device=dev)
+        save_mean = torch.empty(n_domains, c, dtype=torch.float32, device=dev)
+        save_w = torch.empty(n_domains, c // gs, gs, gs, dtype=torch.float32, device=dev)
+        ws = nv.workspace(dev, n, c, h * w, gs, n_domains)
+        rm = nv.ptr_array([p[0] for p in running]) if update else None
+        rv = nv.ptr_array([p[1] for p in running]) if update else None
+        nv_kind = nv.KIND_WHITEN if kind == "whiten" else nv.KIND_BN
+        with torch.cuda.device(dev):
+            rc = lib.dwt_site_pool_fwd(nv_kind, nv.ptr(x), nv.ptr(y), nv.ptr(argmax), n, c, h, w, gs, n_domains, eps, momentum,
+                                       int(update), rm, rv, nv.ptr(gamma_c), nv.ptr(beta_c), nv.ptr(save_mean), nv.ptr(save_w),
+                                       nv.ptr(ws), ws.numel(), nv.stream_ptr(dev))
+        nv.check(rc)
+        nv.poll_status(dev)
+        if update:
+            seen = set()
+            for buf in (t for pair in running for t in pair):
+                if id(buf) not in seen:
+                    seen.add(id(buf))
+                    torch.autograd.graph.increment_version(buf)
+        ctx.save_for_backward(x, argmax, save_mean, save_w, gamma_c, beta_c)
+        ctx.cfg = (nv_kind, gs, n_domains, n, c, h, w, eps, gamma.shape)
+        return y
+
+    @staticmethod
+    def backward(ctx, dy):
+        lib = nv.lib()
+        x, argmax, save_mean, save_w, gamma_c, beta_c = ctx.saved_tensors
+        nv_kind, gs, n_domains, n, c, h, w, eps, gshape = ctx.cfg
+        dy2 = ctx.__dict__.pop("_dwt_extra_grad", None)
+        if dy2 is not None and not (dy2.shape == dy.shape and dy2.dtype == torch.float32
+                                    and dy2.is_contiguous(memory_format=torch.channels_last)):
+            dy, dy2 = dy + dy2, None
+        dy = dy.contiguous(memory_format=torch.channels_last)
+        dev = nv.require_cuda(dy)
+        dsite, dx = torch.empty_like(x), torch.empty_like(x)
+        want_affine = ctx.needs_input_grad[1] or ctx.needs_input_grad[2]
+        dgamma = torch.empty(c, dtype=torch.float32, device=dev) if want_affine else None
+        dbeta = torch.empty(c, dtype=torch.float32, device=dev) if want_affine else None
+        ws = nv.workspace(dev, n, c, h * w, gs, n_domains)
+        with torch.cuda.device(dev):
+            rc = lib.dwt_site_pool_bwd(nv_kind, nv.ptr(x), nv.ptr(dy), nv.ptr(dy2), nv.ptr(argmax), nv.ptr(dsite), nv.ptr(dx), n, c, h, w, gs,
+                                       n_domains, eps, nv.ptr(save_mean), nv.ptr(save_w), nv.ptr(gamma_c), nv.ptr(beta_c),
+                                       nv.ptr(dgamma), nv.ptr(dbeta), nv.ptr(ws), ws.numel(), nv.stream_ptr(dev))
+        nv.check(rc)
+        if want_affine:
+            dgamma, dbeta = dgamma.view(gshape), dbeta.view(gshape)
+        return dx, dgamma, dbeta, None, None, None, None
+
+
+def site_maxpool(x, gamma, beta, *, kind, group_size, n_domains, site):
+    running, eps, momentum, update = site
+    return _SitePoolFunction.apply(x, gamma, beta, kind, group_size, n_domains,
+                                   (running, float(eps), float(momentum), bool(update)))
+
+
 class _ForkForSum(torch.autograd.Function):
 
     @staticmethod
@@ -247,7 +323,8 @@
 
 def fork_for_sum(y):
     fn = getattr(y, "grad_fn", None)
-    if not torch.is_grad_enabled() or fn is None or not isinstance(fn, (_NormFunction._backward_cls, _TailPairFunction._backward_cls)):
+    producers = (_NormFunction._backward_cls, _TailPairFunction._backward_cls, _SitePoolFunction._backward_cls)
+    if not torch.is_grad_enabled() or fn is None or not isinstance(fn, producers):
         return y, y
     return _ForkForSum.apply(y)
 
diff --git a/dwt-domain-adaptation_b200/dwt_b200/fused.py b/dwt-domain-adaptation_b200/dwt_b200/fused.py
--- a/dwt-domain-adaptation_b200/dwt_b200/fused.py
+++ b/dwt-domain-adaptation_b200/dwt_b200/fused.py
@@ -5,6 +5,7 @@
 
 from . import _native as nv
 from . import functional as F
+from .pooling import MaxPool2d
 
 
 class DomainTripleNorm(nn.Module):
@@ -64,6 +65,21 @@
         return F.tail_pair(x, xd, gamma, beta, down_gamma, down_beta, kind=self.kind, group_size=self.group_size,
                            n_domains=self.n_domains, sites=(site_args, down_args))
 
+    def forward_with_maxpool(self, x, domain_modules, gamma, beta, kernel_size, stride, padding, replicated=False,
+                             count_batches=True):
+        mods = list(domain_modules)
+        pooled = (self.kernel_epilogue and not replicated and (kernel_size, stride, padding) == (3, 2, 1)
+                  and len(mods) == self.n_domains and mods[0].training and x.dim() == 4
+                  and x.is_contiguous(memory_format=torch.channels_last) and not x.is_contiguous()
+                  and x.shape[2] % 4 == 0 and x.shape[3] % 4 == 0 and nv.channels_last_supported(x.shape[1], self.group_size))
+        if not pooled:
+            y = self(x, mods, gamma, beta, True, replicated=replicated, count_batches=count_batches)
+            if y.dim() == 4 and y.is_contiguous(memory_format=torch.channels_last) and y.shape[1] % 4 == 0:
+                return MaxPool2d(kernel_size, stride, padding)(y)
+            return torch.nn.functional.max_pool2d(y, kernel_size, stride, padding)
+        return F.site_maxpool(x, gamma, beta, kind=self.kind, group_size=self.group_size, n_domains=self.n_domains,
+                              site=self._running_args(mods, count_batches))
+
     @staticmethod
     def _tensor_epilogue(y, gamma, beta, relu, residual):
         if residual is not None and not relu:
diff --git a/harness/resnet50_dwt.py b/harness/resnet50_dwt.py
--- a/harness/resnet50_dwt.py
+++ b/harness/resnet50_dwt.py
@@ -203,7 +203,14 @@
             self._bump_counters()
         _BATCHED_COUNTERS[0] = batched
         try:
-            x = self.maxpool(self._site("1", self._stem(x), relu=True))
+            stem = getattr(self, "_fused_1", None) if self.training else None
+            if stem is not None and hasattr(stem, "forward_with_maxpool"):
+                names, gname, bname, _ = self._sites["1"]
+                x = stem.forward_with_maxpool(self._stem(x), [getattr(self, n).wh for n in names], getattr(self, gname),
+                                              getattr(self, bname), 3, 2, 1, replicated=_REPLICATED[0],
+                                              count_batches=not _BATCHED_COUNTERS[0])
+            else:
+                x = self.maxpool(self._site("1", self._stem(x), relu=True))
             x = self.layer4(self.layer3(self.layer2(self.layer1(x))))
         finally:
             _BATCHED_COUNTERS[0] = False
diff --git a/include/dwt_b200.h b/include/dwt_b200.h
--- a/include/dwt_b200.h
+++ b/include/dwt_b200.h
@@ -8,7 +8,7 @@
 extern "C" {
 #endif
 
-#define DWT_B200_ABI_VERSION 6
+#define DWT_B200_ABI_VERSION 7
 #define DWT_MAX_DOMAINS 4
 #define DWT_MAX_GROUP_SIZE 64
 
@@ -88,6 +88,15 @@
                   const uint8_t *relu_mask, float *dz, int64_t N, int64_t C, int64_t HW, int group_size,
                   int n_domains, void *workspace, size_t workspace_bytes, dwt_stream_t stream);
 
+DWT_API int dwt_site_pool_fwd(int kind, const float *x, float *y, uint8_t *argmax, int64_t N, int64_t C, int64_t H, int64_t W,
+                      int group_size, int n_domains, float eps, float momentum, int update_running,
+                      float *const *running_mean, float *const *running_cov, const float *gamma, const float *beta,
+                      float *save_mean, float *save_w, void *workspace, size_t workspace_bytes, dwt_stream_t stream);
+DWT_API int dwt_site_pool_bwd(int kind, const float *x, const float *dy, const float *dy2, const uint8_t *argmax, float *dsite,
+                      float *dx, int64_t N, int64_t C, int64_t H, int64_t W, int group_size, int n_domains, float eps,
+                      const float *save_mean, const float *save_w, const float *gamma, const float *beta, float *dgamma,
+                      float *dbeta, void *workspace, size_t workspace_bytes, dwt_stream_t stream);
+
 DWT_API int dwt_mec_fwd_bwd(const float *x, const float *y, int64_t N, int64_t K, float *loss, float *gx,
                     float *gy, dwt_stream_t stream);
 
```

Measured after the change: 2900 (median of 6 runs). About the same (+0.6%).
